# hbaatz/nerf-tex

Hardware: AMD Instinct MI355X
Metric: ray-samples/sec (MLP+composite) at 800x800x64 (higher is better)
Workload: dtype f32; 1 GPU; carpet 800x800x64: 640000 all-hit rays x 64 samples per GPU (BASELINE configs[1]), ParamNerf n_parameters=[1, 6], seeded glorot weights, inputs resident in HBM, fused PE+MLP+composite; rays_per_gpu=640000, hit_rays_total=640000, samples_per_ray=64

## Files before the change

### nerf_tex_amd/csrc/ntx_train.hip

```cpp
#include "nerftex.h"

#include <hip/hip_runtime.h>

#include <algorithm>
#include <cmath>
#include <cstdint>
#include <cstdio>
#include <cstdlib>
#include <cstring>
#include <type_traits>
#include <vector>

#include "ntx_train_device.h"

extern "C" int ntx_set_error(int code, const char *fmt, ...);

#define TRAIN_TRY(expr)                                                                                  \
    do {                                                                                                 \
        hipError_t e_ = (expr);                                                                          \
        if (e_ != hipSuccess) return ntx_set_error(NTX_E_HIP, "%s: %s", #expr, hipGetErrorString(e_)); \
    } while (0)

namespace ntx_train {

constexpr int TM = 128;

struct GemmArgs {
    const float *A; int lda; const float *B; int ldb; float *C; int ldc;
    int M, N, K;
    const float *bias;
    const float *mask; int ldmask;
    int relu, accumulate;
    int k_chunk; long long split_stride;
    float *colsum;
    int aligned;
};

template <int n, bool FAST>
__device__ __forceinline__ void fetch_run(const float *g, bool row_ok, int first, int bound, float *r, bool aligned_ok = false) {
    if (FAST) {
        const f32x4 *v = reinterpret_cast<const f32x4 *>(g);
#pragma unroll
        for (int q = 0; q < n / 4; ++q) { const f32x4 x = v[q]; r[4 * q] = x.x; r[4 * q + 1] = x.y; r[4 * q + 2] = x.z; r[4 * q + 3] = x.w; }
    } else if (row_ok && first + n <= bound && aligned_ok) {
        const f32x4 *v = reinterpret_cast<const f32x4 *>(g);
#pragma unroll
        for (int q = 0; q < n / 4; ++q) { const f32x4 x = v[q]; r[4 * q] = x.x; r[4 * q + 1] = x.y; r[4 * q + 2] = x.z; r[4 * q + 3] = x.w; }
    } else {
#pragma unroll
        for (int q = 0; q < n; ++q) r[q] = (row_ok && first + q < bound) ? g[q] : 0.0f;
    }
}

template <bool A_KCONTIG, int TN_, int TK_>
__device__ __forceinline__ void gemm_body(const GemmArgs &g, int bx, int by, int bz) {
    constexpr int THREADS = TN_ * 2, WCOLS = TN_ / 64, LROWA = TM + 4, LROWB_ = TN_ + 4;
    constexpr int FA = TM * TK_ / THREADS;
    constexpr int FB = TN_ * TK_ / THREADS;
    constexpr int TPR = THREADS / TK_;
    static_assert(FA % 4 == 0 && FB % 4 == 0 && FA * (THREADS / TM) == TK_ && TPR * FB == TN_ && TPR * FA == TM, "panel split");
    __shared__ __attribute__((aligned(16))) float As[2][TK_][LROWA], Bs[2][TK_][LROWB_];
    const int lane = threadIdx.x & 63, wave = threadIdx.x >> 6;
    const int j0 = bx * TN_, i0 = by * TM;
    const int k_begin = bz * g.k_chunk;
    const int k_end = k_begin + g.k_chunk < g.K ? k_begin + g.k_chunk : g.K;
    float *C = g.C + (size_t)bz * (size_t)g.split_stride;
    f32x16 acc[2][2];
#pragma unroll
    for (int a = 0; a < 2; ++a)
#pragma unroll
        for (int b = 0; b < 2; ++b)
#pragma unroll
            for (int r = 0; r < 16; ++r) acc[a][b][r] = 0.0f;
    float ra[2][FA], rb[2][FB], cs[FB];
#pragma unroll
    for (int q = 0; q < FB; ++q) cs[q] = 0.0f;
    const bool want_colsum = !A_KCONTIG && g.colsum != nullptr && by == 0;
    const bool inner = g.aligned && i0 + TM <= g.M && j0 + TN_ <= g.N;
    const int a_row = A_KCONTIG ? (int)(threadIdx.x % TM) : (int)(threadIdx.x / TPR), a_off = A_KCONTIG ? (int)(threadIdx.x / TM) * FA : (int)(threadIdx.x % TPR) * FA;
    const int b_row = (int)(threadIdx.x / TPR), b_off = (int)(threadIdx.x % TPR) * FB;
    auto fetch = [&](int k0, float *fa, float *fb) {
        const bool al = g.aligned != 0;
        if (A_KCONTIG) fetch_run<FA, false>(g.A + (size_t)(i0 + a_row) * g.lda + k0 + a_off, i0 + a_row < g.M, k0 + a_off, k_end, fa, al);
        else fetch_run<FA, false>(g.A + (size_t)(k0 + a_row) * g.lda + i0 + a_off, k0 + a_row < k_end, i0 + a_off, g.M, fa, al);
        fetch_run<FB, false>(g.B + (size_t)(k0 + b_row) * g.ldb + j0 + b_off, k0 + b_row < k_end, j0 + b_off, g.N, fb, al);
    };
    auto stash = [&](int buf, const float *fa, const float *fb) {
        if (want_colsum) {
#pragma unroll
            for (int q = 0; q < FB; ++q) cs[q] += fb[q];
        }
        if (A_KCONTIG) {
#pragma unroll
            for (int q = 0; q < FA; ++q) As[buf][a_off + q][a_row] = fa[q];
        } else {
            f32x4 *d = reinterpret_cast<f32x4 *>(&As[buf][a_row][a_off]);
#pragma unroll
            for (int q = 0; q < FA / 4; ++q) d[q] = f32x4{fa[4 * q], fa[4 * q + 1], fa[4 * q + 2], fa[4 * q + 3]};
        }
        f32x4 *d = reinterpret_cast<f32x4 *>(&Bs[buf][b_row][b_off]);
#pragma unroll
        for (int q = 0; q < FB / 4; ++q) d[q] = f32x4{fb[4 * q], fb[4 * q + 1], fb[4 * q + 2], fb[4 * q + 3]};
    };
    const int n_panels = (k_end - k_begin + TK_ - 1) / TK_;
    const int n_full = inner ? (k_end - k_begin) / TK_ : 0;
    const int wi = (wave / WCOLS) * 64 + 2 * (lane & 31), wj = (wave % WCOLS) * 64 + 2 * (lane & 31), kh = lane >> 5;
    const bool wave_live = j0 + (wave % WCOLS) * 64 < g.N;
    auto compute = [&](int buf) {
        if (!wave_live) return;
        f32x2 av[2], bv[2];
        av[0] = *reinterpret_cast<const f32x2 *>(&As[buf][kh][wi]); bv[0] = *reinterpret_cast<const f32x2 *>(&Bs[buf][kh][wj]);
#pragma unroll
        for (int st = 0; st < TK_ / 2; ++st) {
            const int c = st & 1, n = c ^ 1;
            if (st + 1 < TK_ / 2) {
                const int kk = 2 * (st + 1) + kh;
                av[n] = *reinterpret_cast<const f32x2 *>(&As[buf][kk][wi]); bv[n] = *reinterpret_cast<const f32x2 *>(&Bs[buf][kk][wj]);
            }
            __builtin_amdgcn_sched_barrier(0);
            acc[0][0] = __builtin_amdgcn_mfma_f32_32x32x2f32(av[c].x, bv[c].x, acc[0][0], 0, 0, 0);
            acc[0][1] = __builtin_amdgcn_mfma_f32_32x32x2f32(av[c].x, bv[c].y, acc[0][1], 0, 0, 0);
            acc[1][0] = __builtin_amdgcn_mfma_f32_32x32x2f32(av[c].y, bv[c].x, acc[1][0], 0, 0, 0);
            acc[1][1] = __builtin_amdgcn_mfma_f32_32x32x2f32(av[c].y, bv[c].y, acc[1][1], 0, 0, 0);
            __builtin_amdgcn_sched_barrier(0);
        }
    };
    auto fetch_fast = [&](int k0, float *fa, float *fb) {
        const float *ga = A_KCONTIG ? g.A + (size_t)(i0 + a_row) * g.lda + k0 + a_off : g.A + (size_t)(k0 + a_row) * g.lda + i0 + a_off;
        fetch_run<FA, true>(ga, true, 0, 0, fa);
        fetch_run<FB, true>(g.B + (size_t)(k0 + b_row) * g.ldb + j0 + b_off, true, 0, 0, fb);
    };
    auto pipeline = [&](auto fast_tag, int first, int last) {
        constexpr bool FAST = decltype(fast_tag)::value;
        auto get = [&](int kt, float *fa, float *fb) { if (FAST) fetch_fast(k_begin + kt * TK_, fa, fb); else fetch(k_begin + kt * TK_, fa, fb); };
        if (first >= last) return;
        get(first, ra[0], rb[0]); stash(0, ra[0], rb[0]);
        if (first + 1 < last) get(first + 1, ra[1], rb[1]);
        __syncthreads();
        int kt = first;
        for (; kt + 3 < last; kt += 2) {
            get(kt + 2, ra[0], rb[0]); compute(0); stash(1, ra[1], rb[1]); __syncthreads();
            get(kt + 3, ra[1], rb[1]); compute(1); stash(0, ra[0], rb[0]); __syncthreads();
        }
        for (; kt < last; ++kt) {
            const int buf = (kt - first) & 1;
            if (kt + 2 < last) { if (buf) get(kt + 2, ra[1], rb[1]); else get(kt + 2, ra[0], rb[0]); }
            compute(buf);
            if (kt + 1 < last) { if (buf) stash(0, ra[0], rb[0]); else stash(1, ra[1], rb[1]); }
            __syncthreads();
        }
    };
    pipeline(std::true_type{}, 0, n_full);
    pipeline(std::false_type{}, n_full, n_panels);
    const bool whole = i0 + TM <= g.M && j0 + TN_ <= g.N && (g.ldc % 2 == 0) && (!g.mask || g.ldmask % 2 == 0) && ((uintptr_t)C % 8 == 0) && ((uintptr_t)g.mask % 8 == 0);
    const int j = j0 + (wave % WCOLS) * 64 + 2 * (lane & 31);
    const float bj0 = (g.bias && j < g.N) ? g.bias[j] : 0.0f, bj1 = (g.bias && j + 1 < g.N) ? g.bias[j + 1] : 0.0f;
#pragma unroll
    for (int a = 0; a < 2; ++a)
#pragma unroll
        for (int r = 0; r < 16; ++r) {
            const int i = i0 + (wave / WCOLS) * 64 + 2 * (8 * (r >> 2) + (r & 3) + 4 * kh) + a;
            float v0 = acc[a][0][r], v1 = acc[a][1][r];
            float *c = C + (size_t)i * g.ldc + j;
            if (whole) {
                f32x2 *c2 = reinterpret_cast<f32x2 *>(c);
                if (g.accumulate) { const f32x2 o = *c2; v0 += o.x; v1 += o.y; }
                v0 += bj0; v1 += bj1;
                if (g.relu) { v0 = v0 > 0.0f ? v0 : 0.0f; v1 = v1 > 0.0f ? v1 : 0.0f; }
                if (g.mask) { const f32x2 mk = *reinterpret_cast<const f32x2 *>(g.mask + (size_t)i * g.ldmask + j); if (!(mk.x > 0.0f)) v0 = 0.0f; if (!(mk.y > 0.0f)) v1 = 0.0f; }
                *c2 = f32x2{v0, v1};
            } else if (i < g.M) {
#pragma unroll
                for (int b = 0; b < 2; ++b) {
                    if (j + b >= g.N) continue;
                    float v = b ? v1 : v0;
                    if (g.accumulate) v = v + c[b];
                    v = v + (b ? bj1 : bj0);
                    if (g.relu) v = v > 0.0f ? v : 0.0f;
                    if (g.mask && !(g.mask[(size_t)i * g.ldmask + j + b] > 0.0f)) v = 0.0f;
                    c[b] = v;
                }
            }
        }
    if (want_colsum) {
        float (*red)[LROWB_] = Bs[0];
#pragma unroll
        for (int q = 0; q < FB; ++q) red[b_row][b_off + q] = cs[q];
        __syncthreads();
        if ((int)threadIdx.x < TN_ && j0 + (int)threadIdx.x < g.N) {
            float sum = 0.0f;
            for (int q = 0; q < TK_; ++q) sum += red[q][threadIdx.x];
            g.colsum[(size_t)bz * g.N + j0 + threadIdx.x] = sum;
        }
    }
}


__device__ __forceinline__ void gemm_place(int lin, int nx, int ny, int nz, int &bx, int &by, int &bz) {
    const int tiles = nx * ny;
    if (nz % 8 == 0) {
        const int xcd = lin & 7, slot = lin >> 3, tile = slot % tiles;
        bz = (slot / tiles) * 8 + xcd; bx = tile % nx; by = tile / nx;
    } else { bx = lin % nx; by = (lin / nx) % ny; bz = lin / tiles; }
}
template <bool A_KCONTIG, int TN_, int TK_, int WAVES_PER_EU = 2>
__global__ __launch_bounds__(TN_ * 2) __attribute__((amdgpu_waves_per_eu(WAVES_PER_EU, 8))) void gemm_kernel(GemmArgs g) {
    int bx, by, bz;
    gemm_place(blockIdx.x + gridDim.x * (blockIdx.y + gridDim.y * blockIdx.z), gridDim.x, gridDim.y, gridDim.z, bx, by, bz);
    gemm_body<A_KCONTIG, TN_, TK_>(g, bx, by, bz);
}

constexpr int MAX_REDUCE_BATCH = 32;
struct ReduceJob { const float *partial; int n_split; long long stride, count, pair; float *out; long long first; };
struct ReduceBatch { ReduceJob job[MAX_REDUCE_BATCH]; int n; };
__global__ void reduce_batch_kernel(ReduceBatch b) {
    const long long g = (long long)blockIdx.x * blockDim.x + threadIdx.x;
    int j = 0;
    while (j + 1 < b.n && g >= b.job[j + 1].first) ++j;
    const ReduceJob &r = b.job[j];
    const long long e = g - r.first;
    if (e >= r.count) return;
    float s4[4] = {0.0f, 0.0f, 0.0f, 0.0f};
    auto at = [&](int z) { const float *p = r.partial + (size_t)z * r.stride + e; return r.pair > 0 ? p[0] + p[r.pair] : p[0]; };
    int z = 0;
    for (; z + 4 <= r.n_split; z += 4) {
#pragma unroll
        for (int q = 0; q < 4; ++q) s4[q] += at(z + q);
    }
    for (int q = 0; z < r.n_split; ++z, ++q) s4[q] += at(z);
    r.out[e] = (s4[0] + s4[1]) + (s4[2] + s4[3]);
}

enum { PACK_HIDDEN = 0, PACK_LINEAR = 1, PACK_AUX_ROW = 2, PACK_AUX_RGB = 3, PACK_COPY = 4 };
struct PackSeg {
    const float *src; long long sk, sc;
    int mode;
    int K, ncols, nt;
    float *dst; long long first, count;
};
struct PackArgs { const PackSeg *seg; int n_seg; long long total; };
__global__ void pack_kernel(PackArgs a) {
    const long long e = (long long)blockIdx.x * blockDim.x + threadIdx.x;
    if (e >= a.total) return;
    int lo = 0, hi = a.n_seg - 1;
    while (lo < hi) { const int mid = (lo + hi + 1) >> 1; if (a.seg[mid].first <= e) lo = mid; else hi = mid - 1; }
    const PackSeg &p = a.seg[lo];
    const long long o = e - p.first;
    float v = 0.0f;
    if (p.mode == PACK_COPY) v = p.src[o];
    else if (p.mode == PACK_AUX_ROW) {
        const int h = (int)(o >> 7) & 1, V = (int)(o & 127), k = hidden_row(V, h);
        v = k < p.K ? p.src[k * p.sk] : 0.0f;
    } else if (p.mode == PACK_AUX_RGB) {
        const int c = (int)(o >> 7), h = (int)(o >> 6) & 1, V = (int)(o & 63);
        v = p.src[hidden_row(V, h) * 3 + c];
    } else {
        const int c = (int)(o & 3), lane = (int)((o >> 2) & 63);
        const long long rec = o >> 8;
        const int G = p.nt / 4, g = (int)(rec % G), s = (int)(rec / G);
        const int f = lane & 31, kh = lane >> 5;
        const int k = p.mode == PACK_HIDDEN ? hidden_row(s, kh) : 2 * s + kh, col = 32 * (4 * g + c) + f;
        if (k < p.K && col < p.ncols) v = p.src[k * p.sk + col * p.sc];
    }
    p.dst[o] = v;
}

struct EncodeArgs {
    const float *rays_o, *rays_d, *z, *params, *cone;
    long long rays_per_param_row, M;
    int n_rays, S, n_geo, n_app, pos_freq, dir_freq, param_freq, blur_idx;
    float *posO; int ptiles;
    float *dirO; int dtiles;
    float *dists;
};
__global__ __launch_bounds__(64) void encode_kernel(EncodeArgs a) {
    const int lane = threadIdx.x, n = lane & 31, h = lane >> 5, blk = blockIdx.x, part = blockIdx.y;
    const long long m = (long long)blk * 32 + n;
    const bool valid = m < a.M;
    const int ray = valid ? (int)(m / a.S) : 0, s = valid ? (int)(m - (long long)ray * a.S) : 0;
    const float d[3] = {a.rays_d[3 * ray], a.rays_d[3 * ray + 1], a.rays_d[3 * ray + 2]};
    const float dn = sqrtf((d[0] * d[0] + d[1] * d[1]) + d[2] * d[2]);
    const float zr = a.z[(size_t)ray * a.S + s];
    const bool hit = isfinite(zr);
    const float z = hit ? zr : 0.0f;
    const int P = a.n_geo + a.n_app;
    const float *pr = a.params + (size_t)(ray / a.rays_per_param_row) * (P > 0 ? P : 1);
    auto param = [&](int c) { return c == a.blur_idx ? (hit ? pr[c] * (a.cone[ray] * z) : 0.0f) : pr[c]; };
    float *O = part == 0 ? a.posO : a.dirO;
    const int tiles = part == 0 ? a.ptiles : a.dtiles;
    auto put = [&](int row, float v) {
        if (!valid) v = 0.0f;
        O[(((size_t)blk * tiles + (row >> 5)) * 4 + (n >> 3)) * 256 + ((row & 31) + 32 * ((n >> 2) & 1)) * 4 + (n & 3)] = v;
    };
    auto fourier = [&](int r0, int D, int L, auto x) {
        if (h == 0) for (int c = 0; c < D; ++c) put(r0 + c, x(c));
        for (int f = 0; f < L; ++f)
            for (int c = 0; c < D; ++c) put(r0 + D + 2 * D * f + h * D + c, ntx::sin_q(ldexpf(1.0f, f) * x(c), h));
    };
    if (part == 0) {
        const float o[3] = {a.rays_o[3 * ray], a.rays_o[3 * ray + 1], a.rays_o[3 * ray + 2]};
        fourier(0, 3, a.pos_freq, [&](int c) { return o[c] + d[c] * z; });
        if (a.n_geo > 0) fourier(3 * (1 + 2 * a.pos_freq), a.n_geo, a.param_freq, [&](int c) { return param(c); });
    } else {
        fourier(0, 3, a.dir_freq, [&](int c) { return d[c] / dn; });
        if (a.n_app > 0) fourier(3 * (1 + 2 * a.dir_freq), a.n_app, a.param_freq, [&](int c) { return param(a.n_geo + c); });
        if (valid && h == 0) {
            const float zn = s + 1 < a.S ? a.z[(size_t)ray * a.S + s + 1] : 0.0f;
            const float dist = s + 1 < a.S ? zn - z : (a.S > 1 ? z - a.z[(size_t)ray * a.S + s - 1] : 0.0f);
            a.dists[(size_t)ray * a.S + s] = hit ? dist * dn : 0.0f;
        }
    }
}

__global__ __launch_bounds__(64) void encode_ipe_kernel(EncodeArgs a) {
    const int lane = threadIdx.x, n = lane & 31, h = lane >> 5, blk = blockIdx.x, part = blockIdx.y;
    const long long m = (long long)blk * 32 + n;
    const bool valid = m < a.M;
    const int ray = valid ? (int)(m / a.S) : 0, s = valid ? (int)(m - (long long)ray * a.S) : 0;
    const float d[3] = {a.rays_d[3 * ray], a.rays_d[3 * ray + 1], a.rays_d[3 * ray + 2]};
    const float dn = sqrtf((d[0] * d[0] + d[1] * d[1]) + d[2] * d[2]);
    const float *zr = a.z + (size_t)ray * (a.S + 1) + s;
    const float e0 = zr[0], e1 = zr[1];
    const bool hit = isfinite(e0) && isfinite(e1);
    const int P = a.n_geo + a.n_app;
    const float *pr = a.params + (size_t)(ray / a.rays_per_param_row) * (P + 1);
    auto param = [&](int k) { return pr[k < a.blur_idx ? k : k + 1]; };
    float *O = part == 0 ? a.posO : a.dirO;
    const int tiles = part == 0 ? a.ptiles : a.dtiles;
    auto put = [&](int row, float v) {
        if (!valid) v = 0.0f;
        O[(((size_t)blk * tiles + (row >> 5)) * 4 + (n >> 3)) * 256 + ((row & 31) + 32 * ((n >> 2) & 1)) * 4 + (n & 3)] = v;
    };
    auto fourier = [&](int r0, int D, int L, auto x) {
        if (h == 0) for (int c = 0; c < D; ++c) put(r0 + c, x(c));
        for (int f = 0; f < L; ++f)
            for (int c = 0; c < D; ++c) put(r0 + D + 2 * D * f + h * D + c, ntx::sin_q(ldexpf(1.0f, f) * x(c), h));
    };
    if (part == 0) {
        float mean[3] = {a.rays_o[3 * ray], a.rays_o[3 * ray + 1], a.rays_o[3 * ray + 2]}, cov[3] = {0.0f, 0.0f, 0.0f};
        if (hit) {
            float t_mean, t_var, r_var;
            ntx::cone_moments((e0 + e1) / 2.0f, (e1 - e0) / 2.0f, pr[a.blur_idx] * a.cone[ray], t_mean, t_var, r_var);
            for (int c = 0; c < 3; ++c) mean[c] = mean[c] + d[c] * t_mean;
            ntx::cone_cov(t_var, r_var, d, cov);
        }
        const int L = a.pos_freq;
        for (int f = 0; f < L; ++f)
            for (int c = 0; c < 3; ++c)
                put(h * 3 * L + 3 * f + c, ntx::sin_q(mean[c] * ldexpf(1.0f, f), h) * expf(-0.5f * (cov[c] * ldexpf(1.0f, 2 * f))));
        if (a.n_geo > 0) fourier(6 * L, a.n_geo, a.param_freq, [&](int c) { return param(c); });
    } else {
        fourier(0, 3, a.dir_freq, [&](int c) { return d[c] / dn; });
        if (a.n_app > 0) fourier(3 * (1 + 2 * a.dir_freq), a.n_app, a.param_freq, [&](int c) { return param(a.n_geo + c); });
        if (valid && h == 0) a.dists[(size_t)ray * a.S + s] = hit ? (e1 - e0) * dn : 0.0f;
    }
}

struct DirRowArgs {
    const float *rays_d, *params; long long rays_per_param_row;
    int n_rays, n_geo, n_app, dir_freq, param_freq, Kd, splice;
    const float *w, *bias;
    float *rows;
};
__global__ __launch_bounds__(256) void dirrow_kernel(DirRowArgs a) {
    __shared__ float feat[8 * MAX_PB_GROUPS];
    const int ray = blockIdx.x, f = threadIdx.x;
    const float d[3] = {a.rays_d[3 * ray], a.rays_d[3 * ray + 1], a.rays_d[3 * ray + 2]};
    const float dn = sqrtf((d[0] * d[0] + d[1] * d[1]) + d[2] * d[2]);
    const int P = a.n_geo + a.n_app + (a.splice >= 0 ? 1 : 0);
    const float *pr = a.params + (size_t)(ray / a.rays_per_param_row) * (P > 0 ? P : 1);
    if (f < a.Kd) {
        const int K3 = 3 * (1 + 2 * a.dir_freq);
        const int r = f < K3 ? f : f - K3, D = f < K3 ? 3 : a.n_app;
        auto x = [&](int c) { const int k = a.n_geo + c; return f < K3 ? d[c] / dn : pr[a.splice >= 0 && k >= a.splice ? k + 1 : k]; };
        float v;
        if (r < D) v = x(r);
        else { const int q = r - D, band = q / (2 * D), hc = q - band * 2 * D, hh = hc / D, c = hc - hh * D; v = ntx::sin_q(ldexpf(1.0f, band) * x(c), hh); }
        feat[f] = v;
    }
    __syncthreads();
    float acc = a.bias[f];
    for (int k = 0; k < a.Kd; ++k) acc = fmaf(feat[k], a.w[(size_t)k * 256 + f], acc);
    const int T = f >> 5, g = (f >> 3) & 3, h = (f >> 2) & 1, c = f & 3;
    a.rows[(size_t)ray * 256 + h * 128 + 16 * T + 4 * g + c] = acc;
}

struct CompositeArgs {
    const float *raw_rgb, *sigma, *dists;
    const float *noise;
    int n_rays, S, map_exr, composite_bkgd; float bkgd[3];
    const float *color_true, *alpha_true;
    int kind, loss_fn, alpha_loss_fn, filter_color_loss, use_hard_mask; float gamma;
    float *color, *alpha, *ray_loss;
    float *weights;
    float *dgrad;
    float *dhead;
    long long M;
};
constexpr int MAX_TRAIN_SAMPLES = 1024;
__device__ __forceinline__ float wave_sumf(float v) { for (int o = 32; o > 0; o >>= 1) v += __shfl_xor(v, o); return v; }
__device__ __forceinline__ float rgb_of(float raw, int map_exr) {
    if (map_exr) return raw > 0.0f ? raw + 1.0f : expf(raw);
    return 1.0f / (1.0f + expf(-raw));
}
__device__ __forceinline__ void loss_term(int fn, float t, float p, float inv_n, float &value, float &grad) {
    if (fn == NTX_LOSS_MSE) { const float e = t - p; value = e * e * inv_n; grad = -2.0f * e * inv_n; }
    else {
        const float e = t - p, den = (t + p) + 1e-2f, ae = fabsf(e);
        const float sgn = e > 0.0f ? 1.0f : (e < 0.0f ? -1.0f : 0.0f);
        value = ae / den * inv_n; grad = (-sgn / den - ae / (den * den)) * inv_n;
    }
}
__device__ __forceinline__ size_t dhead_at(long long m, int row) {
    const long long blk = m >> 5; const int p = (int)(m & 31);
    return (size_t)((blk * 4 + (p >> 3)) * 256 + (row + 32 * ((p >> 2) & 1)) * 4 + (p & 3));
}
__global__ __launch_bounds__(256) void composite_loss_kernel(CompositeArgs a) {
    __shared__ float sh_a[4][MAX_TRAIN_SAMPLES], sh_T[4][MAX_TRAIN_SAMPLES];
    const int lane = threadIdx.x & 63, wave = threadIdx.x >> 6;
    if (blockIdx.x == 0) {
        const long long end = (a.M + 31) / 32 * 32;
        for (long long m = a.M + threadIdx.x; m < end; m += 256)
            for (int r = 0; r < 4; ++r) a.dhead[dhead_at(m, r)] = 0.0f;
    }
    const int ray = blockIdx.x * 4 + wave;
    if (ray >= a.n_rays) return;
    const int S = a.S;
    const float *sg = a.sigma + (size_t)ray * S, *ds = a.dists + (size_t)ray * S, *rr = a.raw_rgb + (size_t)ray * S * 3;
    const float *nz = a.noise ? a.noise + (size_t)ray * S : nullptr;
    float *el = sh_a[wave], *T = sh_T[wave];
    for (int s = lane; s < S; s += 64) { const float v = nz ? sg[s] + nz[s] : sg[s]; const float r = v > 0.0f ? v : 0.0f; el[s] = expf(-r * ds[s]); }
    __builtin_amdgcn_wave_barrier();
    float carry = 1.0f;
    for (int s0 = 0; s0 < S; s0 += 64) {
        const int s = s0 + lane;
        float f = s < S ? el[s] + 1e-10f : 1.0f, incl = f;
        for (int o = 1; o < 64; o <<= 1) { const float w = __shfl_up(incl, o); if (lane >= o) incl *= w; }
        float excl = __shfl_up(incl, 1);
        if (lane == 0) excl = 1.0f;
        if (s < S) T[s] = carry * excl;
        carry *= __shfl(incl, 63);
    }
    __builtin_amdgcn_wave_barrier();
    float c0 = 0.0f, c1 = 0.0f, c2 = 0.0f, A = 0.0f;
    for (int s = lane; s < S; s += 64) {
        const float w = (1.0f - el[s]) * T[s];
        c0 += w * rgb_of(rr[3 * s], a.map_exr); c1 += w * rgb_of(rr[3 * s + 1], a.map_exr); c2 += w * rgb_of(rr[3 * s + 2], a.map_exr);
        A += w;
        if (a.weights) a.weights[(size_t)ray * S + s] = w;
    }
    c0 = wave_sumf(c0); c1 = wave_sumf(c1); c2 = wave_sumf(c2); A = wave_sumf(A);
    if (a.composite_bkgd) { c0 += (1.0f - A) * a.bkgd[0]; c1 += (1.0f - A) * a.bkgd[1]; c2 += (1.0f - A) * a.bkgd[2]; }
    const float cp[3] = {c0, c1, c2};
    float dC[3], dA = 0.0f, total = 0.0f;
    {
        const float inv_c = 1.0f / (float)(a.n_rays * 3), inv_a = 1.0f / (float)a.n_rays;
        float mask = 1.0f;
        if (a.kind == NTX_LOSS_ALPHA && a.filter_color_loss) mask = a.use_hard_mask ? (a.alpha_true[ray] > 0.0f ? 1.0f : 0.0f) : a.alpha_true[ray];
        for (int c = 0; c < 3; ++c) {
            float v, gr;
            loss_term(a.loss_fn, a.color_true[3 * ray + c] * mask, cp[c] * mask, inv_c, v, gr);
            total += v; dC[c] = gr * mask;
        }
        if (a.kind == NTX_LOSS_ALPHA) { float v; loss_term(a.alpha_loss_fn, a.alpha_true[ray], A, inv_a, v, dA); total += a.gamma * v; dA *= a.gamma; }
    }
    if (lane == 0) { a.color[3 * ray] = c0; a.color[3 * ray + 1] = c1; a.color[3 * ray + 2] = c2; a.alpha[ray] = A; a.ray_loss[ray] = total; }
    if (a.composite_bkgd) dA -= (dC[0] * a.bkgd[0] + dC[1] * a.bkgd[1]) + dC[2] * a.bkgd[2];
    float Z_carry = 1.0f, V_carry = 0.0f;
    for (int s0 = ((S - 1) / 64) * 64; s0 >= 0; s0 -= 64) {
        const int s = s0 + lane;
        float cs = 0.0f, rgb[3] = {0.0f, 0.0f, 0.0f}, e = 1.0f;
        float F = 1.0f, Bz = 0.0f, Bv = 0.0f;
        if (s < S) {
            e = el[s];
            for (int c = 0; c < 3; ++c) rgb[c] = rgb_of(rr[3 * s + c], a.map_exr);
            cs = (dC[0] * rgb[0] + dC[1] * rgb[1]) + dC[2] * rgb[2];
            F = e + 1e-10f; Bz = -1e-10f; Bv = cs * (1.0f - e);
        }
        for (int o = 1; o < 64; o <<= 1) {
            const float Fo = __shfl_down(F, o), Bzo = __shfl_down(Bz, o), Bvo = __shfl_down(Bv, o);
            if (lane + o < 64) { Bz = fmaf(F, Bzo, Bz); Bv = fmaf(F, Bvo, Bv); F *= Fo; }
        }
        float Fn = __shfl_down(F, 1), Bzn = __shfl_down(Bz, 1), Bvn = __shfl_down(Bv, 1);
        if (lane == 63) { Fn = 1.0f; Bzn = 0.0f; Bvn = 0.0f; }
        const float Z = fmaf(Fn, Z_carry, Bzn), V = fmaf(Fn, V_carry, Bvn);
        if (s < S) {
            const float w = (1.0f - e) * T[s];
            const float d_a = T[s] * fmaf(dA, Z, cs - V);
            const float sig = nz ? sg[s] + nz[s] : sg[s];
            float gr[4];
            for (int c = 0; c < 3; ++c) {
                const float raw = rr[3 * s + c];
                const float drgb = a.map_exr ? (raw > 0.0f ? 1.0f : expf(raw)) : rgb[c] * (1.0f - rgb[c]);
                gr[c] = w * dC[c] * drgb;
            }
            gr[3] = sig > 0.0f ? d_a * ds[s] * e : 0.0f;
            const long long m = (long long)ray * S + s;
            *reinterpret_cast<f32x4 *>(a.dgrad + 4 * m) = f32x4{gr[0], gr[1], gr[2], gr[3]};
            for (int r = 0; r < 4; ++r) a.dhead[dhead_at(m, r)] = gr[r];
        }
        const float F0 = __shfl(F, 0);
        Z_carry = fmaf(F0, Z_carry, __shfl(Bz, 0)); V_carry = fmaf(F0, V_carry, __shfl(Bv, 0));
    }
}
__global__ __launch_bounds__(1024) void loss_sum_kernel(const float *__restrict__ ray_loss, int n_rays, float *__restrict__ loss) {
    __shared__ float red[1024];
    float total = 0.0f;
    for (int r = threadIdx.x; r < n_rays; r += blockDim.x) total += ray_loss[r];
    red[threadIdx.x] = total;
    __syncthreads();
    for (int o = blockDim.x / 2; o > 0; o >>= 1) { if ((int)threadIdx.x < o) red[threadIdx.x] += red[threadIdx.x + o]; __syncthreads(); }
    if (threadIdx.x == 0) *loss = red[0];
}

__global__ void adam_kernel(float *__restrict__ w, const float *__restrict__ g, float *__restrict__ m, float *__restrict__ v, long long n, float lr_t, float b1,
                            float b2, float eps) {
    const long long e = (long long)blockIdx.x * blockDim.x + threadIdx.x;
    if (e >= n) return;
    const float ge = g[e];
    const float me = m[e] + (ge - m[e]) * (1.0f - b1);
    const float ve = v[e] + (ge * ge - v[e]) * (1.0f - b2);
    m[e] = me; v[e] = ve;
    w[e] = w[e] - (me * lr_t) / (sqrtf(ve) + eps);
}

}

struct TLayer { int in, out; size_t w, b; };

struct ntx_trainer {
    int device = 0, cus = 256;
    ntx_model_desc desc{};
    int Kp = 0, Kd = 0, P = 0, ptiles = 0, dtiles = 0, PS = 0, DS = 0;
    bool ipe = false;
    TLayer trunk[8], feature, c1, c2, rgb, alpha;
    size_t n_weights = 0;
    long long cap = 0, cap_blocks = 0, cap_rays = 0;
    float *w = nullptr, *grad = nullptr, *adam_m = nullptr, *adam_v = nullptr;
    float *wfwd = nullptr, *wdx = nullptr, *aux = nullptr; size_t fwd_floats = 0, dx_floats = 0;
    ntx_train::PackSeg *pack_seg = nullptr; int n_pack = 0; long long pack_total = 0;
    float *posO = nullptr, *dirO = nullptr;
    float *act = nullptr; long long act_stride = 0;
    unsigned int *bits = nullptr; long long bits_stride = 0;
    int fwd_variant = 0;
    float *sigma = nullptr, *raw_rgb = nullptr, *z = nullptr, *dists = nullptr, *noise = nullptr;
    float *dirrow = nullptr;
    float *dgrad = nullptr, *dhead = nullptr, *gout = nullptr; long long gout_stride = 0;
    ntx_train::DwJob *jobs = nullptr; int n_jobs = 0; long long total_cost = 0;
    std::vector<ntx_train::DwJob> jobs_host; std::vector<int> reduce_job;
    float *dw_partial = nullptr;
    ntx_train::ReduceBatch reduce{};
    float *color = nullptr, *alpha_out = nullptr, *ray_loss = nullptr, *loss = nullptr;
    float *weights_out = nullptr;
    float *stash = nullptr;
    long long adam_iterations = 0;
};

namespace {

using namespace ntx_train;


void free_all(ntx_trainer *t) {
    if (!t) return;
    (void)hipSetDevice(t->device);
    void *ptrs[] = {t->w, t->grad, t->adam_m, t->adam_v, t->wfwd, t->wdx, t->aux, t->pack_seg, t->posO, t->dirO, t->sigma, t->raw_rgb, t->z, t->dists, t->noise,
                    t->dgrad, t->dhead, t->jobs, t->dw_partial, t->stash, t->dirrow, t->color, t->alpha_out, t->ray_loss, t->loss, t->act, t->bits, t->gout};
    for (void *p : ptrs) if (p) (void)hipFree(p);
    delete t;
}

template <bool AK>
void launch_gemm(hipStream_t st, GemmArgs g) {
    g.k_chunk = g.K;
    g.aligned = (g.lda % 4 == 0) && (g.ldb % 4 == 0) && (((uintptr_t)g.A | (uintptr_t)g.B) % 16 == 0);
    hipLaunchKernelGGL((gemm_kernel<AK, 128, 16>), dim3((g.N + 127) / 128, (g.M + TM - 1) / TM, 1), dim3(256), 0, st, g);
}

}

namespace ntx_train {
template <int K, bool HOIST> void launch_fwd_variant(hipStream_t st, unsigned grid, const FwdArgs &a);
void launch_fwd_chain(int variant, bool hoist, hipStream_t st, unsigned grid, const FwdArgs &a) {
    switch (variant * 2 + (hoist ? 1 : 0)) {
        case 0: launch_fwd_variant<0, false>(st, grid, a); break;
        case 1: launch_fwd_variant<0, true>(st, grid, a); break;
        case 2: launch_fwd_variant<1, false>(st, grid, a); break;
        case 3: launch_fwd_variant<1, true>(st, grid, a); break;
        case 4: launch_fwd_variant<2, false>(st, grid, a); break;
        case 5: launch_fwd_variant<2, true>(st, grid, a); break;
        case 6: launch_fwd_variant<3, false>(st, grid, a); break;
        default: launch_fwd_variant<3, true>(st, grid, a); break;
    }
}
}

extern "C" {

int ntx_sample_depths(const float *t, int64_t n_rays, int n_points, uint32_t flags, uint64_t perturb_seed, const ntx_render_opts *opts, float *z_out,
                      ntx_stream stream);
int ntx_sample_noise(int64_t n_rays, int n_points, uint64_t seed, const ntx_render_opts *opts, float *noise_out, ntx_stream stream);

int ntx_trainer_create(const ntx_model_desc *desc, const float *weights, size_t n_floats, int device, int64_t max_rays, int max_samples_per_ray, ntx_trainer **out) {
    if (!out) return ntx_set_error(NTX_E_INVALID, "out is NULL");
    *out = nullptr;
    if (!desc || !weights) return ntx_set_error(NTX_E_INVALID, "desc / weights is NULL");
    const bool ipe = desc->pos_encoding == NTX_POS_IPE && desc->n_pos == 6;
    if (desc->kind != NTX_MODEL_PARAMNERF || desc->depth != 8 || desc->width != 256 || desc->skip != 4 || desc->color_depth != 1 ||
        !((desc->pos_encoding == NTX_POS_FOURIER && desc->n_pos == 3) || ipe))
        return ntx_set_error(NTX_E_UNSUPPORTED, "training is built for the ParamNerf architecture of the shipped training configs (depth 8, width 256, skips [4], color_depth 1, "
                                                "Fourier features on n_pos 3 or IPE on n_pos 6); others render but do not train");
    if (desc->n_geo < 0 || desc->n_app < 0 || desc->n_geo + desc->n_app > 16) return ntx_set_error(NTX_E_INVALID, "n_parameters out of range");
    if (desc->pos_freq < 0 || desc->dir_freq < 0 || desc->param_freq < 0) return ntx_set_error(NTX_E_INVALID, "negative band count");
    const int Kp = (ipe ? 6 * desc->pos_freq : 3 * (1 + 2 * desc->pos_freq)) + desc->n_geo * (1 + 2 * desc->param_freq), Kd = 3 * (1 + 2 * desc->dir_freq) + desc->n_app * (1 + 2 * desc->param_freq);
    if (Kp > 8 * MAX_PB_GROUPS || Kd > 8 * MAX_PB_GROUPS)
        return ntx_set_error(NTX_E_UNSUPPORTED, "training: pos_map (%d) / dir_map (%d) wider than %d features (the chain holds a block's encoded inputs in registers)", Kp, Kd,
                             8 * MAX_PB_GROUPS);
    if (max_rays < 1 || max_samples_per_ray < 2 || max_samples_per_ray > MAX_TRAIN_SAMPLES || max_rays * (int64_t)max_samples_per_ray > (int64_t)1 << 30)
        return ntx_set_error(NTX_E_INVALID, "max_rays / max_samples_per_ray out of range (samples per ray <= %d)", MAX_TRAIN_SAMPLES);
    int ndev = 0;
    if (hipGetDeviceCount(&ndev) != hipSuccess || ndev <= 0) return ntx_set_error(NTX_E_NODEVICE, "no HIP device visible");
    if (device < 0 || device >= ndev) return ntx_set_error(NTX_E_INVALID, "device %d out of range [0,%d)", device, ndev);
    ntx_trainer *t = new ntx_trainer();
    t->device = device; t->desc = *desc; t->ipe = ipe;
    t->P = desc->n_geo + desc->n_app; t->Kp = Kp; t->Kd = Kd;
    t->ptiles = (Kp + 31) / 32; t->dtiles = (Kd + 31) / 32;
    {
        const int psg = ((Kp + 1) / 2 + 3) / 4, dsg = ((Kd + 1) / 2 + 3) / 4;
        t->fwd_variant = 3;
        for (int v = 2; v >= 0; --v)
            if (FWD_VARIANTS[v][0] >= psg && FWD_VARIANTS[v][1] >= dsg &&
                FWD_VARIANTS[v][0] + FWD_VARIANTS[v][1] <= FWD_VARIANTS[t->fwd_variant][0] + FWD_VARIANTS[t->fwd_variant][1]) t->fwd_variant = v;
        t->PS = 4 * FWD_VARIANTS[t->fwd_variant][0]; t->DS = 4 * FWD_VARIANTS[t->fwd_variant][1];
    }
    size_t p = 0;
    auto take = [&](int in, int o) { TLayer l{in, o, p, p + (size_t)in * o}; p += (size_t)in * o + o; return l; };
    int k = Kp;
    for (int i = 0; i < 8; ++i) { t->trunk[i] = take(k, 256); k = 256 + (i == 4 ? Kp : 0); }
    t->feature = take(256, 256); t->c1 = take(256 + Kd, 256); t->c2 = take(256, 128); t->rgb = take(128, 3); t->alpha = take(256, 1);
    t->n_weights = p;
    if (n_floats != p) { delete t; return ntx_set_error(NTX_E_INVALID, "weights: %zu floats, the model has %zu", n_floats, p); }
    const long long M = (long long)max_rays * max_samples_per_ray, NB = (M + 31) / 32;
    t->cap = M; t->cap_rays = max_rays; t->cap_blocks = NB;
    int rc = hipSetDevice(device) == hipSuccess ? NTX_OK : ntx_set_error(NTX_E_HIP, "hipSetDevice(%d) failed", device);
    if (rc == NTX_OK) { int n = 0; if (hipDeviceGetAttribute(&n, hipDeviceAttributeMultiprocessorCount, device) == hipSuccess && n > 0) t->cus = n; }
    auto alloc = [&](float **d, size_t n, bool zero = false) -> int {
        if (rc != NTX_OK) return rc;
        if (hipMalloc((void **)d, (n ? n : 1) * sizeof(float)) != hipSuccess) return rc = ntx_set_error(NTX_E_HIP, "hipMalloc of %zu floats failed", n);
        if (zero && hipMemset(*d, 0, (n ? n : 1) * sizeof(float)) != hipSuccess) return rc = ntx_set_error(NTX_E_HIP, "hipMemset failed");
        return rc;
    };
    alloc(&t->w, p); alloc(&t->grad, p, true); alloc(&t->adam_m, p, true); alloc(&t->adam_v, p, true);
    alloc(&t->posO, (size_t)NB * t->ptiles * 1024, true); alloc(&t->dirO, (size_t)NB * t->dtiles * 1024, true);
    t->act_stride = t->gout_stride = NB * 8 * 1024; t->bits_stride = NB * 256;
    alloc(&t->act, (size_t)t->act_stride * 11); alloc((float **)&t->bits, (size_t)t->bits_stride * 10); alloc(&t->gout, (size_t)t->gout_stride * 11);
    auto act = [&](int i) { return t->act + (size_t)i * t->act_stride; };
    auto gout = [&](int i) { return t->gout + (size_t)i * t->gout_stride; };
    alloc(&t->sigma, (size_t)M); alloc(&t->raw_rgb, (size_t)M * 3); alloc(&t->z, (size_t)(M + max_rays)); alloc(&t->dists, (size_t)M); alloc(&t->noise, (size_t)M);
    alloc(&t->dirrow, (size_t)max_rays * 256);
    alloc(&t->dgrad, (size_t)NB * 32 * 4); alloc(&t->dhead, (size_t)NB * 1024, true);
    alloc(&t->color, (size_t)max_rays * 3); alloc(&t->alpha_out, (size_t)max_rays); alloc(&t->ray_loss, (size_t)max_rays); alloc(&t->loss, 1);
    if (rc == NTX_OK && hipMemcpy(t->w, weights, p * sizeof(float), hipMemcpyHostToDevice) != hipSuccess) rc = ntx_set_error(NTX_E_HIP, "weight upload failed");
    std::vector<PackSeg> segs;
    long long first = 0;
    auto seg = [&](const float *src, long long sk, long long sc, int mode, int K, int ncols, int nt, size_t *stream_floats, int nsteps) {
        PackSeg s{}; s.src = src; s.sk = sk; s.sc = sc; s.mode = mode; s.K = K; s.ncols = ncols; s.nt = nt;
        const int ring = stream_floats == &t->dx_floats ? DX_RING : RING;
        const long long recs = ((long long)nsteps * (nt / 4) + ring - 1) / ring * ring;
        s.count = recs * 256; s.first = first; s.dst = (float *)(uintptr_t)(*stream_floats * sizeof(float));
        first += s.count; *stream_floats += (size_t)s.count;
        segs.push_back(s);
    };
    const float *W = t->w;
    auto fwd_hidden = [&](const TLayer &l, int row0, int nt) { seg(W + l.w + (size_t)row0 * l.out, l.out, 1, PACK_HIDDEN, 256, l.out, nt, &t->fwd_floats, 128); };
    auto fwd_linear = [&](const TLayer &l, int K, int nsteps) { seg(W + l.w, l.out, 1, PACK_LINEAR, K, l.out, 8, &t->fwd_floats, nsteps); };
    fwd_linear(t->trunk[0], Kp, t->PS);
    for (int i = 1; i < 8; ++i) {
        if (i == 5) { fwd_linear(t->trunk[5], Kp, t->PS); fwd_hidden(t->trunk[5], Kp, 8); }
        else fwd_hidden(t->trunk[i], 0, 8);
    }
    fwd_hidden(t->feature, 0, 8);
    fwd_linear(t->c1, Kd, t->DS); fwd_hidden(t->c1, Kd, 8);
    fwd_hidden(t->c2, 0, 4);
    const size_t n_fwd_segs = segs.size();
    auto dx_hidden = [&](const TLayer &l, int row0, int K, int nsteps) { seg(W + l.w + (size_t)row0 * l.out, 1, l.out, PACK_HIDDEN, K, 256, 8, &t->dx_floats, nsteps); };
    seg(W + t->rgb.w, 1, 3, PACK_LINEAR, 3, 128, 4, &t->dx_floats, 2);
    dx_hidden(t->c2, 0, 128, 64);
    dx_hidden(t->c1, Kd, 256, 128);
    dx_hidden(t->feature, 0, 256, 128);
    seg(W + t->alpha.w, 1, 1, PACK_LINEAR, 1, 256, 8, &t->dx_floats, 1);
    for (int i = 7; i >= 1; --i) dx_hidden(t->trunk[i], i == 5 ? Kp : 0, 256, 128);
    const size_t n_stream_segs = segs.size();
    auto tail = [&](size_t of, size_t *stream_floats) { PackSeg s = segs[of]; s.count = (long long)(stream_floats == &t->dx_floats ? DX_RING : RING) * 256; s.first = first; s.dst = (float *)(uintptr_t)(*stream_floats * sizeof(float));
                                                        first += s.count; *stream_floats += (size_t)s.count; segs.push_back(s); };
    tail(0, &t->fwd_floats); tail(n_fwd_segs, &t->dx_floats);
    auto aux_seg = [&](const float *src, int mode, int K, long long count, size_t at) {
        PackSeg s{}; s.src = src; s.sk = 1; s.mode = mode; s.K = K; s.count = count; s.first = first; s.dst = (float *)(uintptr_t)(at * sizeof(float));
        first += count; segs.push_back(s);
    };
    for (int i = 0; i < 8; ++i) aux_seg(W + t->trunk[i].b, PACK_AUX_ROW, 256, 256, AUX_BIAS + (size_t)i * 256);
    aux_seg(W + t->feature.b, PACK_AUX_ROW, 256, 256, AUX_BIAS + 8 * 256); aux_seg(W + t->c1.b, PACK_AUX_ROW, 256, 256, AUX_BIAS + 9 * 256);
    aux_seg(W + t->c2.b, PACK_AUX_ROW, 128, 256, AUX_BIAS + 10 * 256);
    aux_seg(W + t->alpha.w, PACK_AUX_ROW, 256, 256, AUX_ALPHA_W); aux_seg(W + t->alpha.b, PACK_COPY, 1, 1, AUX_ALPHA_B);
    aux_seg(W + t->rgb.w, PACK_AUX_RGB, 128, 384, AUX_RGB_W); aux_seg(W + t->rgb.b, PACK_COPY, 3, 3, AUX_RGB_B);
    t->pack_total = first; t->n_pack = (int)segs.size();
    alloc(&t->wfwd, t->fwd_floats); alloc(&t->wdx, t->dx_floats); alloc(&t->aux, AUX_FLOATS, true);
    if (rc == NTX_OK) {
        for (size_t i = 0; i < segs.size(); ++i) {
            const bool is_aux = i >= n_stream_segs + 2, is_fwd = i < n_fwd_segs || i == n_stream_segs;
            float *base = is_aux ? t->aux : is_fwd ? t->wfwd : t->wdx;
            segs[i].dst = (float *)((char *)base + (uintptr_t)segs[i].dst);
        }
        if (hipMalloc((void **)&t->pack_seg, segs.size() * sizeof(PackSeg)) != hipSuccess ||
            hipMemcpy(t->pack_seg, segs.data(), segs.size() * sizeof(PackSeg), hipMemcpyHostToDevice) != hipSuccess)
            rc = ntx_set_error(NTX_E_HIP, "segment table upload failed");
    }
    std::vector<DwJob> &jobs = t->jobs_host;
    struct RJ { int job; long long at, count, pair; size_t out; };
    std::vector<RJ> rjobs;
    auto new_job = [&]() { DwJob j{}; for (DwWave &w : j.w) w.shape = -1; jobs.push_back(j); return (int)jobs.size() - 1; };
    auto matrix = [&](int j, int K, int N, size_t g_kernel, long long g_bias, long long *at_bias) {
        const long long at = jobs[j].slot_floats;
        jobs[j].slot_floats += (long long)K * N;
        rjobs.push_back(RJ{j, at, (long long)K * N, 0, g_kernel});
        *at_bias = -1;
        if (g_bias >= 0) { *at_bias = jobs[j].slot_floats; jobs[j].slot_floats += 2 * N; rjobs.push_back(RJ{j, *at_bias, N, N, (size_t)g_bias}); }
        return at;
    };
    auto wave = [&](int j, int w, int shape, const float *A, int rtA, int a0, const float *B, int rtB, int b0, long long at, int K, int N, int c_lo, long long at_bias) {
        DwWave &d = jobs[j].w[w];
        d.A = A; d.rtA = rtA; d.a0 = a0; d.B = B; d.rtB = rtB; d.b0 = b0; d.shape = shape; d.out = at; d.ldc = N; d.row0 = a0 * 32; d.rows_valid = K;
        d.col0 = b0 * 32; d.c_lo = c_lo; d.c_hi = c_lo + N; d.bias_out = a0 == 0 ? at_bias : -1;
        const int cost = shape == 0 ? 256 : shape == 1 ? 198 : 68;
        if (cost > jobs[j].cost) jobs[j].cost = cost;
    };
    auto layer_job = [&](const float *X, const float *dY, size_t g_kernel, size_t g_bias) {
        const int j = new_job(); long long ab; const long long at = matrix(j, 256, 256, g_kernel, (long long)g_bias, &ab);
        for (int w = 0; w < 4; ++w) wave(j, w, 0, X, 8, 4 * (w >> 1), dY, 8, 4 * (w & 1), at, 256, 256, 0, ab);
    };
    {
        const TLayer &r = t->rgb, &al = t->alpha, &c2 = t->c2, &c1 = t->c1, &f = t->feature;
        for (int i = 7; i >= 1; --i) layer_job(act(i - 1), gout(10 - i), t->trunk[i].w + (size_t)(i == 5 ? Kp : 0) * 256, t->trunk[i].b);
        layer_job(act(7), gout(2), f.w, f.b);
        layer_job(act(8), gout(1), c1.w + (size_t)Kd * 256, c1.b);
        {
            const int j = new_job(); long long ab0, ab5;
            const long long at0 = matrix(j, Kp, 256, t->trunk[0].w, (long long)t->trunk[0].b, &ab0), at5 = matrix(j, Kp, 256, t->trunk[5].w, -1, &ab5);
            for (int w = 0; w < 2; ++w) { wave(j, w, 1, t->posO, t->ptiles, 0, gout(10), 8, 4 * w, at0, Kp, 256, 0, ab0); wave(j, 2 + w, 1, t->posO, t->ptiles, 0, gout(5), 8, 4 * w, at5, Kp, 256, 0, ab5); }
        }
        {
            const int j = new_job(); long long abd, ab2;
            const long long atd = matrix(j, Kd, 256, c1.w, -1, &abd), at2 = matrix(j, 256, 128, c2.w, (long long)c2.b, &ab2);
            for (int w = 0; w < 2; ++w) { wave(j, w, 1, t->dirO, t->dtiles, 0, gout(1), 8, 4 * w, atd, Kd, 256, 0, abd); wave(j, 2 + w, 0, act(9), 8, 4 * w, gout(0), 4, 0, at2, 256, 128, 0, ab2); }
        }
        {
            const int j = new_job(); long long abr, aba;
            const long long atr = matrix(j, 128, 3, r.w, (long long)r.b, &abr), ata = matrix(j, 256, 1, al.w, (long long)al.b, &aba);
            wave(j, 0, 2, act(10), 4, 0, t->dhead, 1, 0, atr, 128, 3, 0, abr);
            for (int w = 0; w < 2; ++w) wave(j, 1 + w, 2, act(7), 8, 4 * w, t->dhead, 1, 0, ata, 256, 1, 3, aba);
        }
    }
    t->n_jobs = (int)jobs.size();
    size_t partial_floats = 0;
    for (DwJob &j : jobs) {
        t->total_cost += j.cost;
    }
    for (DwJob &j : jobs) {
        const long long slots = ((long long)j.cost * t->cus + t->total_cost - 1) / t->total_cost + 2;
        j.first_float = (long long)partial_floats; partial_floats += (size_t)(slots * j.slot_floats);
    }
    alloc(&t->dw_partial, partial_floats);
    if (rc == NTX_OK) {
        if (hipMalloc((void **)&t->jobs, jobs.size() * sizeof(DwJob)) != hipSuccess ||
            hipMemcpy(t->jobs, jobs.data(), jobs.size() * sizeof(DwJob), hipMemcpyHostToDevice) != hipSuccess)
            rc = ntx_set_error(NTX_E_HIP, "job table upload failed");
        if ((int)rjobs.size() > MAX_REDUCE_BATCH) rc = ntx_set_error(NTX_E_INVALID, "trainer: too many weight gradients for one launch");
        long long rfirst = 0;
        for (size_t i = 0; i < rjobs.size() && rc == NTX_OK; ++i) {
            ReduceJob &r = t->reduce.job[t->reduce.n++];
            const DwJob &j = jobs[rjobs[i].job];
            r.partial = t->dw_partial + j.first_float + rjobs[i].at; r.n_split = 0; r.stride = j.slot_floats; r.count = rjobs[i].count; r.pair = rjobs[i].pair;
            r.out = t->grad + rjobs[i].out; r.first = rfirst;
            rfirst += (rjobs[i].count + 255) / 256 * 256;
            t->reduce_job.push_back(rjobs[i].job);
        }
    }
    if (rc != NTX_OK) { free_all(t); return rc; }
    *out = t;
    return NTX_OK;
}

int ntx_trainer_destroy(ntx_trainer *t) { free_all(t); return NTX_OK; }

size_t ntx_trainer_weight_count(const ntx_trainer *t) { return t ? t->n_weights : 0; }

static float *trainer_vector(ntx_trainer *t, int what) {
    return what == NTX_TRAINER_WEIGHTS ? t->w : what == NTX_TRAINER_GRADIENTS ? t->grad : what == NTX_TRAINER_ADAM_M ? t->adam_m : what == NTX_TRAINER_ADAM_V ? t->adam_v : nullptr;
}

int ntx_trainer_get(ntx_trainer *t, int what, float *out_host, size_t n_floats) {
    if (!t || !out_host) return ntx_set_error(NTX_E_INVALID, "NULL argument");
    if (n_floats != t->n_weights) return ntx_set_error(NTX_E_INVALID, "%zu floats asked, the model has %zu", n_floats, t->n_weights);
    const float *src = trainer_vector(t, what);
    if (!src) return ntx_set_error(NTX_E_INVALID, "what = %d", what);
    TRAIN_TRY(hipSetDevice(t->device));
    TRAIN_TRY(hipDeviceSynchronize());
    TRAIN_TRY(hipMemcpy(out_host, src, n_floats * sizeof(float), hipMemcpyDeviceToHost));
    return NTX_OK;
}

int ntx_trainer_activation(ntx_trainer *t, int layer, int64_t n_samples_total, float *out_host) {
    if (!t || !out_host) return ntx_set_error(NTX_E_INVALID, "NULL argument");
    if (n_samples_total < 1 || n_samples_total > t->cap) return ntx_set_error(NTX_E_INVALID, "n_samples_total out of range");
    const float *src = nullptr; int tiles = 8;
    auto act = [&](int i) { return t->act + (size_t)i * t->act_stride; };
    auto gout = [&](int i) { return t->gout + (size_t)i * t->gout_stride; };
    if (layer >= 0 && layer < 8) src = act(layer);
    else if (layer == 8) src = act(9);
    else if (layer == 9) { src = act(10); tiles = 4; }
    else if (layer == 10) src = t->sigma;
    else if (layer >= 20 && layer < 28) src = gout(10 - (layer - 20));
    else if (layer == 28) src = gout(1);
    else if (layer == 29) src = gout(2);
    else if (layer == 11) src = t->raw_rgb;
    else if (layer == 30) src = t->dgrad;
    else return ntx_set_error(NTX_E_INVALID, "layer %d (0-7 trunk, 8 / 9 the colour layers, 10 the density, 11 the raw colour; 20-29 the kept gradients, 30 the composite's adjoint)", layer);
    TRAIN_TRY(hipSetDevice(t->device));
    TRAIN_TRY(hipDeviceSynchronize());
    if (layer == 10 || layer == 11 || layer == 30) {
        const size_t width = layer == 10 ? 1 : (layer == 11 ? 3 : 4);
        TRAIN_TRY(hipMemcpy(out_host, src, (size_t)n_samples_total * width * sizeof(float), hipMemcpyDeviceToHost)); return NTX_OK;
    }
    const long long nb = (n_samples_total + 31) / 32;
    std::vector<float> tmp((size_t)nb * tiles * 1024);
    TRAIN_TRY(hipMemcpy(tmp.data(), src, tmp.size() * sizeof(float), hipMemcpyDeviceToHost));
    const int width = tiles * 32;
    for (long long m = 0; m < n_samples_total; ++m) {
        const long long blk = m >> 5; const int p = (int)(m & 31);
        const float *rec = tmp.data() + ((size_t)blk * tiles * 4 + (p >> 3)) * 256 + 32 * ((p >> 2) & 1) * 4 + (p & 3);
        float *o = out_host + (size_t)m * width;
        for (int T = 0; T < tiles; ++T)
            for (int i = 0; i < 32; ++i) o[32 * T + i] = rec[(size_t)T * 1024 + i * 4];
    }
    return NTX_OK;
}

int ntx_trainer_set_weights(ntx_trainer *t, const float *weights_host, size_t n_floats) { return ntx_trainer_set(t, NTX_TRAINER_WEIGHTS, weights_host, n_floats); }

int ntx_trainer_set(ntx_trainer *t, int what, const float *values_host, size_t n_floats) {
    if (!t || !values_host) return ntx_set_error(NTX_E_INVALID, "NULL argument");
    if (n_floats != t->n_weights) return ntx_set_error(NTX_E_INVALID, "%zu floats given, the model has %zu", n_floats, t->n_weights);
    float *dst = trainer_vector(t, what);
    if (!dst) return ntx_set_error(NTX_E_INVALID, "what = %d", what);
    TRAIN_TRY(hipSetDevice(t->device));
    TRAIN_TRY(hipDeviceSynchronize());
    TRAIN_TRY(hipMemcpy(dst, values_host, n_floats * sizeof(float), hipMemcpyHostToDevice));
    return NTX_OK;
}

int ntx_trainer_set_iterations(ntx_trainer *t, int64_t iterations) {
    if (!t || iterations < 0) return ntx_set_error(NTX_E_INVALID, "trainer is NULL or iterations < 0");
    t->adam_iterations = iterations;
    return NTX_OK;
}

int ntx_trainer_composite_weights(ntx_trainer *t, float *weights_dev) {
    if (!t) return ntx_set_error(NTX_E_INVALID, "trainer is NULL");
    if (t->ipe && weights_dev) return ntx_set_error(NTX_E_UNSUPPORTED, "an IPE trainer has no importance pass (MipRenderer: renderer.py:403-404)");
    t->weights_out = weights_dev;
    return NTX_OK;
}

namespace ntx_train {
__global__ void add_kernel(float *__restrict__ dst, const float *__restrict__ src, long long n) {
    const long long e = (long long)blockIdx.x * blockDim.x + threadIdx.x;
    if (e < n) dst[e] += src[e];
}
}

int ntx_trainer_stash_gradients(ntx_trainer *t, int op, ntx_stream stream) {
    if (!t || (op != 0 && op != 1)) return ntx_set_error(NTX_E_INVALID, "trainer is NULL or op is not 0 (keep) / 1 (add back)");
    TRAIN_TRY(hipSetDevice(t->device));
    if (!t->stash) {
        if (op == 1) return ntx_set_error(NTX_E_INVALID, "no gradient was kept");
        TRAIN_TRY(hipMalloc((void **)&t->stash, t->n_weights * sizeof(float)));
    }
    if (op == 0) TRAIN_TRY(hipMemcpyAsync(t->stash, t->grad, t->n_weights * sizeof(float), hipMemcpyDeviceToDevice, (hipStream_t)stream));
    else hipLaunchKernelGGL(ntx_train::add_kernel, dim3((unsigned)((t->n_weights + 255) / 256)), dim3(256), 0, (hipStream_t)stream, t->grad, t->stash, (long long)t->n_weights);
    TRAIN_TRY(hipGetLastError());
    return NTX_OK;
}

int ntx_trainer_device_weights(ntx_trainer *t, const float **weights_dev) {
    if (!t || !weights_dev) return ntx_set_error(NTX_E_INVALID, "NULL argument");
    *weights_dev = t->w;
    return NTX_OK;
}

int ntx_trainer_allreduce_gradients(ntx_trainer *t, ntx_comm *comm, ntx_stream stream) {
    if (!t || !comm) return ntx_set_error(NTX_E_INVALID, "NULL argument");
    return ntx_allreduce_mean_f32(comm, t->grad, t->n_weights, stream);
}

int ntx_train_step_gradients(ntx_trainer *t, const float *rays_o, const float *rays_d, const float *tnear_far, const float *params, int64_t rays_per_param_row,
                             const float *cone_scale, int64_t n_rays, int n_samples, int blur_idx, uint32_t flags, const float *bkgd, uint64_t perturb_seed,
                             const ntx_render_opts *opts, const float *z_vals, const float *color_true, const float *alpha_true, const ntx_loss_desc *loss,
                             float *color_pred, float *alpha_pred, float *loss_out, ntx_stream stream) {
    if (!t) return ntx_set_error(NTX_E_INVALID, "trainer is NULL");
    const int P_in = t->P + (t->ipe ? 1 : 0);
    if (!rays_o || !rays_d || (!tnear_far && !z_vals) || !color_true || !loss || (P_in > 0 && !params)) return ntx_set_error(NTX_E_INVALID, "NULL buffer");
    if (n_rays < 1 || n_rays > t->cap_rays || n_samples < 2 || (long long)n_rays * n_samples > t->cap) return ntx_set_error(NTX_E_INVALID, "n_rays x n_samples beyond what the trainer was created for");
    if (n_samples > MAX_TRAIN_SAMPLES) return ntx_set_error(NTX_E_INVALID, "n_samples > %d", MAX_TRAIN_SAMPLES);
    if (blur_idx >= P_in || (blur_idx >= 0 && !cone_scale) || (t->ipe && blur_idx < 0)) return ntx_set_error(NTX_E_INVALID, "bad blur_idx / cone_scale");
    if (loss->size < sizeof(ntx_loss_desc) || (loss->kind != NTX_LOSS_NERF && loss->kind != NTX_LOSS_ALPHA) || (loss->loss_fn != NTX_LOSS_MSE && loss->loss_fn != NTX_LOSS_SMAPE) ||
        (loss->alpha_loss_fn != NTX_LOSS_MSE && loss->alpha_loss_fn != NTX_LOSS_SMAPE))
        return ntx_set_error(NTX_E_INVALID, "bad ntx_loss_desc");
    if (loss->kind == NTX_LOSS_ALPHA && !alpha_true) return ntx_set_error(NTX_E_INVALID, "AlphaLoss needs alpha_true");
    if (rays_per_param_row < 1) rays_per_param_row = 1;
    TRAIN_TRY(hipSetDevice(t->device));
    hipStream_t st = (hipStream_t)stream;
    const long long M = (long long)n_rays * n_samples;
    const int S = n_samples, n_blocks = (int)((M + 31) / 32);
    {
        PackArgs pa{t->pack_seg, t->n_pack, t->pack_total};
        hipLaunchKernelGGL(pack_kernel, dim3((unsigned)((t->pack_total + 255) / 256)), dim3(256), 0, st, pa);
    }
    const float *z = z_vals;
    if (!z) {
        int rc = ntx_sample_depths(tnear_far, n_rays, t->ipe ? S + 1 : S, flags & NTX_FLAG_PERTURB, perturb_seed, opts, t->z, stream);
        if (rc != NTX_OK) return rc;
        z = t->z;
    }
    const float *noise = nullptr;
    if (flags & NTX_FLAG_RAW_NOISE) {
        int rc = ntx_sample_noise(n_rays, S, perturb_seed, opts, t->noise, stream);
        if (rc != NTX_OK) return rc;
        noise = t->noise;
    }
    {
        EncodeArgs e{}; e.rays_o = rays_o; e.rays_d = rays_d; e.z = z; e.params = params; e.cone = cone_scale; e.rays_per_param_row = rays_per_param_row; e.M = M;
        e.n_rays = (int)n_rays; e.S = S; e.n_geo = t->desc.n_geo; e.n_app = t->desc.n_app; e.pos_freq = t->desc.pos_freq; e.dir_freq = t->desc.dir_freq;
        e.param_freq = t->desc.param_freq; e.blur_idx = blur_idx; e.posO = t->posO; e.ptiles = t->ptiles; e.dirO = t->dirO;
        e.dtiles = t->dtiles; e.dists = t->dists;
        if (t->ipe) hipLaunchKernelGGL(encode_ipe_kernel, dim3((unsigned)n_blocks, 2), dim3(64), 0, st, e);
        else hipLaunchKernelGGL(encode_kernel, dim3((unsigned)n_blocks, 2), dim3(64), 0, st, e);
    }
    const unsigned chain_grid = (unsigned)std::min<long long>(t->cus, (n_blocks + 3) / 4);
    {
        FwdArgs f{}; f.stream = t->wfwd; f.stream_bytes = (uint32_t)(t->fwd_floats * sizeof(float)); f.aux = t->aux; f.M = M;
        f.ptiles = t->ptiles; f.dtiles = t->dtiles; f.pos = t->posO; f.dir = t->dirO;
        f.act = t->act; f.act_stride = t->act_stride; f.bits = t->bits; f.bits_stride = t->bits_stride;
        f.sigma = t->sigma; f.raw_rgb = t->raw_rgb;
        const bool hoist = (t->ipe || blur_idx < 0 || blur_idx < t->desc.n_geo) && S % 32 == 0 && getenv("NERFTEX_TRAIN_NO_DIR_HOIST") == nullptr;
        if (hoist) {
            DirRowArgs dr{}; dr.rays_d = rays_d; dr.params = params; dr.rays_per_param_row = rays_per_param_row; dr.n_rays = (int)n_rays; dr.n_geo = t->desc.n_geo;
            dr.n_app = t->desc.n_app; dr.dir_freq = t->desc.dir_freq; dr.param_freq = t->desc.param_freq; dr.Kd = t->Kd; dr.w = t->w + t->c1.w; dr.bias = t->w + t->c1.b;
            dr.rows = t->dirrow; dr.splice = t->ipe ? blur_idx : -1;
            hipLaunchKernelGGL(dirrow_kernel, dim3((unsigned)n_rays), dim3(256), 0, st, dr);
        }
        f.dirrow = t->dirrow; f.n_rays = (int)n_rays; f.S = S;
        launch_fwd_chain(t->fwd_variant, hoist, st, chain_grid, f);
    }
    {
        CompositeArgs c{};
        c.raw_rgb = t->raw_rgb; c.sigma = t->sigma; c.dists = t->dists; c.noise = noise; c.n_rays = (int)n_rays; c.S = S; c.map_exr = (flags & NTX_FLAG_MAP_EXR) ? 1 : 0;
        c.composite_bkgd = (flags & NTX_FLAG_COMPOSITE_BKGD) ? 1 : 0;
        for (int k = 0; k < 3; ++k) c.bkgd[k] = bkgd ? bkgd[k] : 1.0f;
        c.color_true = color_true; c.alpha_true = alpha_true; c.kind = loss->kind; c.loss_fn = loss->loss_fn; c.alpha_loss_fn = loss->alpha_loss_fn;
        c.filter_color_loss = loss->filter_color_loss; c.use_hard_mask = loss->use_hard_mask; c.gamma = loss->gamma;
        c.weights = t->weights_out;
        c.color = color_pred ? color_pred : t->color; c.alpha = alpha_pred ? alpha_pred : t->alpha_out; c.ray_loss = t->ray_loss; c.dgrad = t->dgrad; c.dhead = t->dhead; c.M = M;
        hipLaunchKernelGGL(composite_loss_kernel, dim3((unsigned)((n_rays + 3) / 4)), dim3(256), 0, st, c);
        hipLaunchKernelGGL(loss_sum_kernel, dim3(1), dim3(1024), 0, st, t->ray_loss, (int)n_rays, loss_out ? loss_out : t->loss);
    }
    {
        DxArgs d{}; d.stream = t->wdx; d.stream_bytes = (uint32_t)(t->dx_floats * sizeof(float)); d.M = M; d.dgrad = t->dgrad;
        d.out = t->gout; d.out_stride = t->gout_stride; d.bits = t->bits; d.bits_stride = t->bits_stride;
        launch_dx_chain(st, chain_grid, d);
    }
    {
        DwArgs d{}; d.jobs = t->jobs; d.n_jobs = t->n_jobs; d.n_blocks = n_blocks; d.total_cost = t->total_cost; d.partial = t->dw_partial;
        const long long G = t->cus, W = t->total_cost * n_blocks;
#ifdef NTX_TRAIN_CLOCKS
        static unsigned long long *clocks = nullptr;
        const size_t nck = (size_t)G * (2 + 3 * t->n_jobs);
        if (getenv("NERFTEX_DW_CLOCKS")) {
            if (!clocks) (void)hipMalloc((void **)&clocks, nck * sizeof(unsigned long long));
            (void)hipMemsetAsync(clocks, 0, nck * sizeof(unsigned long long), st);
            d.clocks = clocks;
        }
#endif
        launch_dw(st, (unsigned)G, d);
#ifdef NTX_TRAIN_CLOCKS
        if (d.clocks) {
            std::vector<unsigned long long> h(nck);
            (void)hipStreamSynchronize(st);
            (void)hipMemcpy(h.data(), clocks, nck * sizeof(unsigned long long), hipMemcpyDeviceToHost);
            unsigned long long t0 = ~0ull;
            for (long long g = 0; g < G; ++g) t0 = std::min(t0, h[g * (2 + 3 * t->n_jobs)]);
            FILE *f = fopen(getenv("NERFTEX_DW_CLOCKS"), "w");
            if (f) {
                for (long long g = 0; g < G; ++g) {
                    const unsigned long long *c = &h[g * (2 + 3 * t->n_jobs)];
                    fprintf(f, "%lld %llu %llu", g, c[0] - t0, c[1] - t0);
                    for (int j = 0; j < t->n_jobs; ++j) if (c[4 + 3 * j]) fprintf(f, "  j%d cost %d blocks %llu %llu-%llu", j, t->jobs_host[j].cost, c[2 + 3 * j], c[3 + 3 * j] - t0, c[4 + 3 * j] - t0);
                    fprintf(f, "\n");
                }
                fclose(f);
            }
        }
#endif
        ReduceBatch rb = t->reduce;
        std::vector<int> slots(t->n_jobs);
        long long start = 0;
        for (int j = 0; j < t->n_jobs; ++j) {
            const long long span = (long long)t->jobs_host[j].cost * n_blocks;
            slots[j] = (int)(dw_last_g(G, W, start, span) - dw_first_g(G, W, start) + 1);
            start += span;
        }
        for (int i = 0; i < rb.n; ++i) rb.job[i].n_split = slots[t->reduce_job[i]];
        const long long total = rb.job[rb.n - 1].first + (rb.job[rb.n - 1].count + 255) / 256 * 256;
        hipLaunchKernelGGL(reduce_batch_kernel, dim3((unsigned)(total / 256)), dim3(256), 0, st, rb);
    }
    TRAIN_TRY(hipGetLastError());
    return NTX_OK;
}

int ntx_trainer_adam_step(ntx_trainer *t, float lrate, float lrate_decay_steps, float lrate_decay_rate, float beta_1, float beta_2, float epsilon, ntx_stream stream) {
    if (!t) return ntx_set_error(NTX_E_INVALID, "trainer is NULL");
    TRAIN_TRY(hipSetDevice(t->device));
    const double step = (double)t->adam_iterations;
    double lr = lrate;
    if (lrate_decay_steps > 0) lr = (double)lrate * std::pow((double)lrate_decay_rate, step / (double)lrate_decay_steps);
    const double tt = step + 1.0;
    const float lr_t = (float)((double)(float)lr * std::sqrt(1.0 - std::pow((double)beta_2, tt)) / (1.0 - std::pow((double)beta_1, tt)));
    hipLaunchKernelGGL(ntx_train::adam_kernel, dim3((unsigned)((t->n_weights + 255) / 256)), dim3(256), 0, (hipStream_t)stream, t->w, t->grad, t->adam_m, t->adam_v,
                       (long long)t->n_weights, lr_t, beta_1, beta_2, epsilon);
    t->adam_iterations += 1;
    TRAIN_TRY(hipGetLastError());
    return NTX_OK;
}

int64_t ntx_trainer_iterations(const ntx_trainer *t) { return t ? t->adam_iterations : -1; }

int ntx_gemm_f32(const float *A, int lda, int a_kcontig, const float *B, int ldb, int b_kcontig, float *C, int ldc, int M, int N, int K, const float *bias, int relu,
                 ntx_stream stream) {
    if (!A || !B || !C || M < 1 || N < 1 || K < 1) return ntx_set_error(NTX_E_INVALID, "bad GEMM arguments");
    ntx_train::GemmArgs g{}; g.A = A; g.lda = lda; g.B = B; g.ldb = ldb; g.C = C; g.ldc = ldc; g.M = M; g.N = N; g.K = K; g.bias = bias; g.relu = relu;
    hipStream_t st = (hipStream_t)stream;
    if (b_kcontig) return ntx_set_error(NTX_E_UNSUPPORTED, "B must be [K][N]");
    if (a_kcontig) launch_gemm<true>(st, g); else launch_gemm<false>(st, g);
    TRAIN_TRY(hipGetLastError());
    return NTX_OK;
}

}
```

### nerf_tex_amd/csrc/ntx_train_device.h

```cpp
#pragma once

#include "ntx_device.h"

namespace ntx_train {

using ntx::f32x16;
using ntx::f32x4;
using ntx::hidden_row;
using ntx::mfma32;
using ntx::RING;
using ntx::static_for;
typedef float f32x2 __attribute__((ext_vector_type(2)));
typedef int i32x4 __attribute__((ext_vector_type(4)));
typedef unsigned int u32x4 __attribute__((ext_vector_type(4)));

#define TRN_DEV __device__ __forceinline__

TRN_DEV __amdgpu_buffer_rsrc_t make_rsrc(const void *base, long long bytes) {
    const long long b = bytes < 0 ? 0 : (bytes > 0x7ffffff0ll ? 0x7ffffff0ll : bytes);
    return __builtin_amdgcn_make_buffer_rsrc(const_cast<void *>(base), 0, (int)b, 0x00020000);
}

TRN_DEV uint32_t o_lane_bytes(int lane) {
    const int n = lane & 31, h = lane >> 5;
    return (uint32_t)((n >> 3) * 1024 + ((n >> 2) & 1) * 512 + h * 64 + (n & 3) * 4);
}
constexpr int STORE_NT = 0;
constexpr uint32_t o_value_bytes(int V) { return (uint32_t)((V >> 4) * 4096 + ((V & 15) >> 2) * 128 + (V & 3) * 16); }

template <int R>
struct WRingT {
    static constexpr int DEPTH = R;
    __amdgpu_buffer_rsrc_t rsrc;
    uint32_t voff;
    f32x4 r[R];
};
typedef WRingT<RING> WRing;
constexpr int DX_RING = 16;
template <class WR>
TRN_DEV f32x4 wr_load(const WR &w, uint32_t byte_off) {
#ifdef NTX_X_WSMALL
    byte_off &= 0xffffu;
#endif
#ifdef NTX_X_NOWLOAD
    if (byte_off >= (uint32_t)WR::DEPTH * 1024u) return w.r[(byte_off >> 10) % WR::DEPTH];
#endif
    return __builtin_bit_cast(f32x4, __builtin_amdgcn_raw_buffer_load_b128(w.rsrc, w.voff, byte_off, 0));
}

template <int NSTEPS, int NMT, bool ZERO, class WR, class Extra>
TRN_DEV void seg_hidden(f32x16 (&acc)[8], WR &ws, uint32_t &sbase, const float (&hin)[128], Extra &&extra) {
    constexpr int RPS = NMT / 4, RING = WR::DEPTH;
    static_assert((NSTEPS * RPS) % RING == 0, "whole ring turns");
    const f32x16 zero = {0.f, 0.f, 0.f, 0.f, 0.f, 0.f, 0.f, 0.f, 0.f, 0.f, 0.f, 0.f, 0.f, 0.f, 0.f, 0.f};
    static_for<NSTEPS>([&](auto S) {
        constexpr int s = S;
        f32x4 w;
        static_for<NMT>([&](auto MT) {
            constexpr int mt = MT;
            if constexpr (mt % 4 == 0) {
                constexpr int rec = s * RPS + mt / 4;
                w = ws.r[rec % RING];
                ws.r[rec % RING] = wr_load(ws, sbase + (uint32_t)(rec + RING) * 1024u);
            }
            if constexpr (ZERO && s == 0) acc[mt] = mfma32(w[mt % 4], hin[s], zero);
            else acc[mt] = mfma32(w[mt % 4], hin[s], acc[mt]);
            extra(S, MT);
            __builtin_amdgcn_sched_barrier(0);
        });
    });
    sbase += (uint32_t)(NSTEPS * RPS) * 1024u;
}

template <int NG, class Fetch>
TRN_DEV void seg_mem(f32x16 (&acc)[8], WRing &ws, uint32_t &sbase, float (&pb)[12], Fetch &&fetch) {
    static_assert(RING == 8, "a group of 4 k-steps of 8 tiles is one ring turn");
    static_for<NG>([&](auto G) {
        constexpr int g = G;
        if constexpr (g + 2 < NG) fetch(std::integral_constant<int, g + 2>{});
        static_for<4>([&](auto K) {
            constexpr int k = K;
            f32x4 w;
            static_for<8>([&](auto MT) {
                constexpr int mt = MT;
                if constexpr (mt % 4 == 0) {
                    constexpr int slot = 2 * k + mt / 4;
                    w = ws.r[slot];
                    ws.r[slot] = wr_load(ws, sbase + (uint32_t)(8 * g + slot + RING) * 1024u);
                }
                acc[mt] = mfma32(w[mt % 4], pb[4 * (g % 3) + k], acc[mt]);
                __builtin_amdgcn_sched_barrier(0);
            });
        });
    });
    sbase += (uint32_t)NG * 8192u;
}

template <int NKS, int NMT, bool ZERO, class WR>
TRN_DEV void seg_few(f32x16 (&acc)[8], WR &ws, uint32_t &sbase, const float (&b)[NKS]) {
    constexpr int RPS = NMT / 4, RING = WR::DEPTH;
    static_assert(NKS * RPS <= RING, "one ring turn");
    const f32x16 zero = {0.f, 0.f, 0.f, 0.f, 0.f, 0.f, 0.f, 0.f, 0.f, 0.f, 0.f, 0.f, 0.f, 0.f, 0.f, 0.f};
    static_for<RING>([&](auto I) {
        constexpr int rec = I;
        const f32x4 w = ws.r[rec];
        ws.r[rec] = wr_load(ws, sbase + (uint32_t)(rec + RING) * 1024u);
        if constexpr (rec < NKS * RPS) {
            constexpr int s = rec / RPS, t0 = 4 * (rec % RPS);
            static_for<4>([&](auto C) {
                constexpr int c = C;
                if constexpr (ZERO && s == 0) acc[t0 + c] = mfma32(w[c], b[s], zero);
                else acc[t0 + c] = mfma32(w[c], b[s], acc[t0 + c]);
                __builtin_amdgcn_sched_barrier(0);
            });
        }
    });
    sbase += (uint32_t)RING * 1024u;
}

template <int V0>
TRN_DEV void convert8_relu_bits(float (&hin)[128], const f32x16 (&prev)[8], uint32_t &w) {
    constexpr int T = V0 >> 4, R = V0 & 15;
    float t0, t1, t2, t3;
    asm("v_accvgpr_read_b32 %0, %13\n\tv_accvgpr_read_b32 %1, %14\n\tv_accvgpr_read_b32 %2, %15\n\tv_accvgpr_read_b32 %3, %16\n\t"
        "v_accvgpr_read_b32 %4, %17\n\tv_accvgpr_read_b32 %5, %18\n\tv_accvgpr_read_b32 %6, %19\n\tv_accvgpr_read_b32 %7, %20\n\t"
        "v_sub_f32 %9, 0, %0\n\tv_sub_f32 %10, 0, %1\n\tv_sub_f32 %11, 0, %2\n\tv_sub_f32 %12, 0, %3\n\t"
        "v_alignbit_b32 %8, %8, %9, 31\n\tv_alignbit_b32 %8, %8, %10, 31\n\tv_alignbit_b32 %8, %8, %11, 31\n\tv_alignbit_b32 %8, %8, %12, 31\n\t"
        "v_sub_f32 %9, 0, %4\n\tv_sub_f32 %10, 0, %5\n\tv_sub_f32 %11, 0, %6\n\tv_sub_f32 %12, 0, %7\n\t"
        "v_alignbit_b32 %8, %8, %9, 31\n\tv_alignbit_b32 %8, %8, %10, 31\n\tv_alignbit_b32 %8, %8, %11, 31\n\tv_alignbit_b32 %8, %8, %12, 31\n\t"
        "v_max_f32 %0, 0, %0\n\tv_max_f32 %1, 0, %1\n\tv_max_f32 %2, 0, %2\n\tv_max_f32 %3, 0, %3\n\t"
        "v_max_f32 %4, 0, %4\n\tv_max_f32 %5, 0, %5\n\tv_max_f32 %6, 0, %6\n\tv_max_f32 %7, 0, %7"
        : "=&v"(hin[V0 + 0]), "=&v"(hin[V0 + 1]), "=&v"(hin[V0 + 2]), "=&v"(hin[V0 + 3]), "=&v"(hin[V0 + 4]), "=&v"(hin[V0 + 5]), "=&v"(hin[V0 + 6]),
          "=&v"(hin[V0 + 7]), "+v"(w), "=&v"(t0), "=&v"(t1), "=&v"(t2), "=&v"(t3)
        : "a"(prev[T][R + 0]), "a"(prev[T][R + 1]), "a"(prev[T][R + 2]), "a"(prev[T][R + 3]), "a"(prev[T][R + 4]), "a"(prev[T][R + 5]), "a"(prev[T][R + 6]),
          "a"(prev[T][R + 7]));
}
constexpr int keep_bit(int V) { return 31 - (V & 31); }

template <int NMT>
TRN_DEV void convert_relu_bits(float (&hin)[128], const f32x16 (&prev)[8], u32x4 &bits) {
    static_for<(NMT + 1) / 2>([&](auto W) {
        constexpr int wd = W;
        uint32_t w = 0;
        static_for<(NMT - 2 * wd >= 2 ? 4 : 2)>([&](auto Q) { convert8_relu_bits<32 * wd + 8 * decltype(Q)::value>(hin, prev, w); });
        bits[wd] = w;
    });
}
template <int NMT>
TRN_DEV void convert_linear(float (&hin)[128], const f32x16 (&prev)[8]) {
    static_for<NMT * 16>([&](auto V) { constexpr int v = V; hin[v] = prev[v >> 4][v & 15]; });
}
template <int NMT>
TRN_DEV void convert_mask(float (&hin)[128], const f32x16 (&prev)[8], const u32x4 &bits) {
    static_for<NMT * 16>([&](auto V) {
        constexpr int v = V;
        const float x = prev[v >> 4][v & 15];
        const int keep = __builtin_amdgcn_sbfe((int)bits[v >> 5], keep_bit(v), 1);
        hin[v] = __builtin_bit_cast(float, __builtin_bit_cast(int, x) & keep);
    });
}

constexpr int AUX_BIAS = 0, AUX_ALPHA_W = 11 * 256, AUX_ALPHA_B = AUX_ALPHA_W + 256, AUX_RGB_W = AUX_ALPHA_B + 4, AUX_RGB_B = AUX_RGB_W + 384,
              AUX_FLOATS = AUX_RGB_B + 4;
template <int MT>
TRN_DEV void bias_tile(f32x16 (&acc)[8], const float *aux, int layer, int h) {
    const f32x4 *b = reinterpret_cast<const f32x4 *>(aux + AUX_BIAS + layer * 256 + h * 128) + MT * 4;
    const f32x4 v0 = b[0], v1 = b[1], v2 = b[2], v3 = b[3];
    acc[MT] = f32x16{v0.x, v0.y, v0.z, v0.w, v1.x, v1.y, v1.z, v1.w, v2.x, v2.y, v2.z, v2.w, v3.x, v3.y, v3.z, v3.w};
}

constexpr int MAX_PB_GROUPS = 12;
struct FwdArgs {
    const float *stream; uint32_t stream_bytes;
    const float *aux;
    long long M;
    int ptiles, dtiles;
    const float *pos, *dir;
    float *act; long long act_stride;
    unsigned int *bits; long long bits_stride;
    float *sigma, *raw_rgb;
    const float *dirrow; int n_rays, S;
};

#ifdef NTX_TRAIN_FWD
template <int PSG, int DSG, bool HOIST>
__global__ __launch_bounds__(256) __attribute__((amdgpu_waves_per_eu(1, 1))) void fwd_chain_kernel(FwdArgs a) {
    __shared__ __attribute__((aligned(16))) float aux_lds[AUX_FLOATS];
    __shared__ __attribute__((aligned(16))) float rows_lds[HOIST ? 4 * 256 : 4];
    ntx::load_aux(aux_lds, a.aux, AUX_FLOATS);
    const int lane = threadIdx.x & 63, n = lane & 31, h = lane >> 5;
    const int wave = __builtin_amdgcn_readfirstlane(blockIdx.x * 4 + (threadIdx.x >> 6)), nwaves = gridDim.x * 4;
    const int n_blocks = (int)((a.M + 31) >> 5);
    if (wave >= n_blocks) return;
    WRing ws;
    ws.rsrc = make_rsrc(a.stream, a.stream_bytes);
    ws.voff = (uint32_t)lane * 16u;
    static_for<RING>([&](auto I) { ws.r[I] = wr_load(ws, (uint32_t)decltype(I)::value * 1024u); });
    const uint32_t lane_o = o_lane_bytes(lane), lane_r = (uint32_t)((n >> 3) * 1024 + ((n >> 2) & 1) * 512 + (n & 3) * 4 + h * 16), lane16 = (uint32_t)lane * 16u;
    float pb[12];
    const __amdgpu_buffer_rsrc_t rs_row = make_rsrc(a.dirrow, HOIST ? (long long)a.n_rays * 1024 : 0);
    __amdgpu_buffer_rsrc_t rs_in = make_rsrc(a.pos + (size_t)wave * a.ptiles * 1024, (long long)a.ptiles * 4096);
    auto fetch = [&](auto G) {
        constexpr int g = G;
        static_for<4>([&](auto K) {
            constexpr int k = K;
            constexpr int s = 4 * g + k;
            pb[4 * (g % 3) + k] = __builtin_bit_cast(float, __builtin_amdgcn_raw_buffer_load_b32(rs_in, lane_r, (uint32_t)((s >> 4) * 4096 + (s & 15) * 32), 0));
        });
    };
    fetch(std::integral_constant<int, 0>{}); fetch(std::integral_constant<int, 1>{});
    for (int blk = wave; blk < n_blocks; blk += nwaves) {
        uint32_t opaque_zero = 0;
        asm volatile("" : "+v"(opaque_zero));
        const float *aux = aux_lds + opaque_zero;
        const float *rows_aux = rows_lds + opaque_zero + (HOIST ? (threadIdx.x >> 6) * 256 : 0) - AUX_BIAS - 9 * 256;
        uint32_t sbase = 0;
        f32x16 acc[8];
        float hin[128];
        const long long m = (long long)blk * 32 + n;
        const bool valid = m < a.M;
        if constexpr (HOIST) {
            const uint32_t ray = __builtin_amdgcn_readfirstlane((int)(((uint32_t)blk * 32u) / (uint32_t)a.S));
            const f32x4 x0 = __builtin_bit_cast(f32x4, __builtin_amdgcn_raw_buffer_load_b128(rs_row, lane16, (ray < (uint32_t)a.n_rays ? ray : (uint32_t)a.n_rays - 1u) * 1024u, 0));
            *reinterpret_cast<f32x4 *>(rows_lds + (threadIdx.x >> 6) * 256 + lane * 4) = x0;
            __builtin_amdgcn_wave_barrier();
        }
        __amdgpu_buffer_rsrc_t rs_out = make_rsrc(a.act, 0);
        auto leaves_to = [&](int idx, int tiles) { rs_out = make_rsrc(a.act + (size_t)idx * a.act_stride + (size_t)blk * tiles * 1024, (long long)tiles * 4096); };
        auto leave = [&](auto V) {
            constexpr int v = V;
#ifndef NTX_X_NOSTORE
            __builtin_amdgcn_raw_buffer_store_b32(__builtin_bit_cast(int, hin[v]), rs_out, lane_o, o_value_bytes(v), STORE_NT);
#endif
        };
        auto bits_leave = [&](int idx, const u32x4 &bw) {
#ifndef NTX_X_NOBITS
            const __amdgpu_buffer_rsrc_t rb = make_rsrc(a.bits + (size_t)idx * a.bits_stride + (size_t)blk * 256, 1024);
            __builtin_amdgcn_raw_buffer_store_b128(__builtin_bit_cast(i32x4, bw), rb, lane16, 0, 0);
#endif
        };
        static_for<8>([&](auto T) { bias_tile<decltype(T)::value>(acc, aux, 0, h); });
        seg_mem<PSG>(acc, ws, sbase, pb, fetch);
        float sig_part = 0.0f;
        auto layer = [&](auto LIc) {
            f32x16 (&cur)[8] = acc; f32x16 (&prev)[8] = acc;
            constexpr int LI = decltype(LIc)::value, in_idx = LI - 1;
            constexpr bool relu_in = in_idx != 8;
            u32x4 bw = {0u, 0u, 0u, 0u};
            if constexpr (HOIST && LI == 9) {
                sbase += (uint32_t)DSG * 8192u;
                static_for<RING>([&](auto I) { ws.r[I] = wr_load(ws, sbase + (uint32_t)decltype(I)::value * 1024u); });
            }
            static_for<4>([&](auto W) {
                constexpr int wd = W;
                if constexpr (relu_in) {
                    uint32_t w = 0;
                    static_for<4>([&](auto Q) { convert8_relu_bits<32 * wd + 8 * decltype(Q)::value>(hin, prev, w); });
                    bw[wd] = w;
                } else static_for<32>([&](auto V) { constexpr int v = 32 * wd + decltype(V)::value; hin[v] = prev[v >> 4][v & 15]; });
                const float *bsrc = (HOIST && LI == 9) ? rows_aux : aux;
                if constexpr (LI < 10 || wd < 2) { bias_tile<2 * wd>(cur, bsrc, LI, h); bias_tile<2 * wd + 1>(cur, bsrc, LI, h); }
            });
            if constexpr (relu_in) bits_leave(in_idx < 8 ? in_idx : 8, bw);
            if constexpr (LI == 8) {
                const f32x4 *wa = reinterpret_cast<const f32x4 *>(aux + AUX_ALPHA_W + h * 128);
                static_for<32>([&](auto I) {
                    constexpr int i = I;
                    const f32x4 w = wa[i];
                    sig_part = __builtin_fmaf(hin[4 * i + 0], w.x, sig_part); sig_part = __builtin_fmaf(hin[4 * i + 1], w.y, sig_part);
                    sig_part = __builtin_fmaf(hin[4 * i + 2], w.z, sig_part); sig_part = __builtin_fmaf(hin[4 * i + 3], w.w, sig_part);
                });
            }
            __builtin_amdgcn_sched_barrier(0);
            leaves_to(in_idx, 8);
            if constexpr (LI == 5) seg_mem<PSG>(cur, ws, sbase, pb, fetch);
            if constexpr (LI == 9 && !HOIST) seg_mem<DSG>(cur, ws, sbase, pb, fetch);
            if constexpr (LI == 4) rs_in = make_rsrc(a.pos + (size_t)blk * a.ptiles * 1024, (long long)a.ptiles * 4096);
            if constexpr (LI == 8 && !HOIST) rs_in = make_rsrc(a.dir + (size_t)blk * a.dtiles * 1024, (long long)a.dtiles * 4096);
            if constexpr (LI == 10) {
                const int nb = blk + nwaves < n_blocks ? blk + nwaves : blk;
                rs_in = make_rsrc(a.pos + (size_t)nb * a.ptiles * 1024, (long long)a.ptiles * 4096);
            }
            auto extra = [&](auto S, auto MT) {
                constexpr int s = decltype(S)::value, mt = decltype(MT)::value;
                if constexpr ((LI == 4 || (LI == 8 && !HOIST) || LI == 10) && mt == 2 && (s == 8 || s == 24)) fetch(std::integral_constant<int, (s == 8 ? 0 : 1)>{});
                if constexpr (mt == 5 || (LI == 10 && mt == 3)) leave(S);
            };
            if constexpr (LI == 10) seg_hidden<128, 4, false>(cur, ws, sbase, hin, extra);
            else seg_hidden<128, 8, false>(cur, ws, sbase, hin, extra);
        };
        static_for<10>([&](auto I) { layer(std::integral_constant<int, decltype(I)::value + 1>{}); });
        {
            u32x4 bw = {0u, 0u, 0u, 0u};
            convert_relu_bits<4>(hin, acc, bw);
            bits_leave(9, bw);
            leaves_to(10, 4);
            static_for<64>([&](auto V) { leave(V); });
            float rgb[3];
            static_for<3>([&](auto C) {
                constexpr int c = C;
                const f32x4 *wc = reinterpret_cast<const f32x4 *>(aux + AUX_RGB_W + (c * 2 + h) * 64);
                float p = 0.0f;
                static_for<16>([&](auto I) {
                    constexpr int i = I;
                    const f32x4 w = wc[i];
                    p = __builtin_fmaf(hin[4 * i + 0], w.x, p); p = __builtin_fmaf(hin[4 * i + 1], w.y, p);
                    p = __builtin_fmaf(hin[4 * i + 2], w.z, p); p = __builtin_fmaf(hin[4 * i + 3], w.w, p);
                });
                rgb[c] = p + __shfl_xor(p, 32, 64) + aux[AUX_RGB_B + c];
            });
            const float sigma = sig_part + __shfl_xor(sig_part, 32, 64) + aux[AUX_ALPHA_B];
            if (valid && h == 0) {
                a.sigma[m] = sigma;
                a.raw_rgb[3 * m + 0] = rgb[0]; a.raw_rgb[3 * m + 1] = rgb[1]; a.raw_rgb[3 * m + 2] = rgb[2];
            }
        }
    }
}

#endif

struct DxArgs {
    const float *stream; uint32_t stream_bytes;
    long long M;
    const float *dgrad;
    float *out; long long out_stride;
    const unsigned int *bits; long long bits_stride;
};

#ifdef NTX_TRAIN_DX
__global__ __launch_bounds__(256) __attribute__((amdgpu_waves_per_eu(1, 1))) void dx_chain_kernel(DxArgs a) {
    const int lane = threadIdx.x & 63, n = lane & 31, h = lane >> 5;
    const int wave = __builtin_amdgcn_readfirstlane(blockIdx.x * 4 + (threadIdx.x >> 6)), nwaves = gridDim.x * 4;
    const int n_blocks = (int)((a.M + 31) >> 5);
    if (wave >= n_blocks) return;
    WRingT<DX_RING> ws;
    ws.rsrc = make_rsrc(a.stream, a.stream_bytes);
    ws.voff = (uint32_t)lane * 16u;
    static_for<DX_RING>([&](auto I) { ws.r[I] = wr_load(ws, (uint32_t)decltype(I)::value * 1024u); });
    const uint32_t lane_o = o_lane_bytes(lane), lane16 = (uint32_t)lane * 16u;
    auto fetch_grad = [&](int blk) {
        const long long m = (long long)blk * 32 + n;
        const f32x4 zero = {0.0f, 0.0f, 0.0f, 0.0f};
        return m < a.M ? *reinterpret_cast<const f32x4 *>(a.dgrad + 4 * m) : zero;
    };
    f32x4 g = fetch_grad(wave);
    for (int blk = wave; blk < n_blocks; blk += nwaves) {
        uint32_t sbase = 0;
        f32x16 acc[8];
        float hin[128];
        __amdgpu_buffer_rsrc_t rs_out = make_rsrc(a.out, 0);
        auto leaves_to = [&](int idx, int tiles) { rs_out = make_rsrc(a.out + (size_t)idx * a.out_stride + (size_t)blk * tiles * 1024, (long long)tiles * 4096); };
        auto leave = [&](auto V) {
            constexpr int v = V;
            __builtin_amdgcn_raw_buffer_store_b32(__builtin_bit_cast(int, hin[v]), rs_out, lane_o, o_value_bytes(v), STORE_NT);
        };
        auto fetch_bits = [&](int idx) {
            const __amdgpu_buffer_rsrc_t rb = make_rsrc(a.bits + (size_t)idx * a.bits_stride + (size_t)blk * 256, 1024);
            return __builtin_bit_cast(u32x4, __builtin_amdgcn_raw_buffer_load_b128(rb, lane16, 0, 0));
        };
        u32x4 bw = fetch_bits(9);
        const float gs = h ? 0.0f : g.w;
        {
            const float b[2] = {h ? g.y : g.x, h ? 0.0f : g.z};
            seg_few<2, 4, true>(acc, ws, sbase, b);
        }
        {
            const int nb = blk + nwaves < n_blocks ? blk + nwaves : blk;
            g = fetch_grad(nb);
        }
        convert_mask<4>(hin, acc, bw);
        bw = fetch_bits(8);
        leaves_to(0, 4);
        seg_hidden<64, 8, true>(acc, ws, sbase, hin, [&](auto S, auto MT) { if constexpr (decltype(MT)::value == 5) leave(S); });
        convert_mask<8>(hin, acc, bw);
        leaves_to(1, 8);
        seg_hidden<128, 8, true>(acc, ws, sbase, hin, [&](auto S, auto MT) { if constexpr (decltype(MT)::value == 5) leave(S); });
        convert_linear<8>(hin, acc);
        static_for<8>([&](auto J) {
            constexpr int j = J;
            bw = fetch_bits(7 - j);
            leaves_to(2 + j, 8);
            seg_hidden<128, 8, true>(acc, ws, sbase, hin, [&](auto S, auto MT) { if constexpr (decltype(MT)::value == 5) leave(S); });
            if constexpr (j == 0) {
                const float b[1] = {gs};
                seg_few<1, 8, false>(acc, ws, sbase, b);
            }
            convert_mask<8>(hin, acc, bw);
        });
        leaves_to(10, 8);
        static_for<128>([&](auto V) { leave(V); });
    }
}

#endif

struct DwWave {
    const float *A; int rtA, a0;
    const float *B; int rtB, b0;
    int shape;
    long long out; int ldc;
    int row0, rows_valid, col0, c_lo, c_hi;
    long long bias_out;
};
struct DwJob { DwWave w[4]; int cost; long long slot_floats, first_float; };
struct DwArgs { const DwJob *jobs; int n_jobs, n_blocks; long long total_cost; float *partial;
                unsigned long long *clocks; };

__host__ __device__ inline long long dw_cut(long long g, long long G, long long W, long long start, long long cost, long long n_blocks) {
    const long long x = g * W / G - start;
    long long b = x <= 0 ? 0 : (x + cost / 2) / cost;
    return b > n_blocks ? n_blocks : b;
}
__host__ __device__ inline long long dw_first_g(long long G, long long W, long long start) { return start * G / W; }
__host__ __device__ inline long long dw_last_g(long long G, long long W, long long start, long long span) { return (start + span - 1) * G / W; }

#ifdef NTX_TRAIN_DW
#ifndef NTX_DW_SYNC
#define NTX_DW_SYNC 16
#endif
constexpr int DW_SYNC = NTX_DW_SYNC;
template <int NA, int NB>
TRN_DEV void dw_piece(const DwWave &tg, float *slot, int blk0, int blk1, int lane) {
    auto uniform_ptr = [](const float *p) {
        const uint32_t lo = (uint32_t)__builtin_amdgcn_readfirstlane((int)(uint32_t)(uintptr_t)p), hi = (uint32_t)__builtin_amdgcn_readfirstlane((int)(uint32_t)((uintptr_t)p >> 32));
        return (const float *)(uintptr_t)(((uint64_t)hi << 32) | (uint64_t)lo);
    };
    const float *A = uniform_ptr(tg.A), *B = uniform_ptr(tg.B);
    const int rtA = __builtin_amdgcn_readfirstlane(tg.rtA), a0 = __builtin_amdgcn_readfirstlane(tg.a0), rtB = __builtin_amdgcn_readfirstlane(tg.rtB), b0 = __builtin_amdgcn_readfirstlane(tg.b0);
    f32x16 acc[NA][NB];
    static_for<NA>([&](auto Ai) { static_for<NB>([&](auto Bi) {
        acc[Ai][Bi] = f32x16{0.f, 0.f, 0.f, 0.f, 0.f, 0.f, 0.f, 0.f, 0.f, 0.f, 0.f, 0.f, 0.f, 0.f, 0.f, 0.f}; }); });
    f32x4 bsum[NB];
    static_for<NB>([&](auto Bi) { bsum[Bi] = f32x4{0.0f, 0.0f, 0.0f, 0.0f}; });
    const bool want_bias = tg.bias_out >= 0;
    const int nblk = blk1 - blk0;
    if (nblk > 0) {
        const __amdgpu_buffer_rsrc_t ra = make_rsrc(A + (size_t)blk0 * rtA * 1024, (long long)nblk * rtA * 4096);
        const __amdgpu_buffer_rsrc_t rb = make_rsrc(B + (size_t)blk0 * rtB * 1024, (long long)nblk * rtB * 4096);
        const uint32_t voff = (uint32_t)lane * 16u;
        const uint32_t stepA = (uint32_t)rtA * 4096u, stepB = (uint32_t)rtB * 4096u, offA = (uint32_t)a0 * 4096u, offB = (uint32_t)b0 * 4096u;
        f32x4 xa[2][NA][2], xb[2][NB][2];
        auto fetch = [&](auto BUF, int i) {
            constexpr int buf = BUF;
#ifdef NTX_X_DWSMALL
            i &= 3;
#endif
#ifdef NTX_X_DWNOLOAD
            if (i > 0) return;
#endif
            const uint32_t oa = (uint32_t)i * stepA + offA + (uint32_t)buf * 2048u, ob = (uint32_t)i * stepB + offB + (uint32_t)buf * 2048u;
            static_for<NA>([&](auto Ai) { static_for<2>([&](auto Q) {
                xa[buf][Ai][Q] = __builtin_bit_cast(f32x4, __builtin_amdgcn_raw_buffer_load_b128(ra, voff, oa + (uint32_t)(decltype(Ai)::value * 4 + decltype(Q)::value) * 1024u, 0)); }); });
            static_for<NB>([&](auto Bi) { static_for<2>([&](auto Q) {
                xb[buf][Bi][Q] = __builtin_bit_cast(f32x4, __builtin_amdgcn_raw_buffer_load_b128(rb, voff, ob + (uint32_t)(decltype(Bi)::value * 4 + decltype(Q)::value) * 1024u, 0)); }); });
        };
        auto compute = [&](auto BUF) {
            constexpr int buf = BUF;
            static_for<2>([&](auto Q) { static_for<4>([&](auto C) {
                constexpr int q = Q, c = C;
                static_for<NA>([&](auto Ai) { static_for<NB>([&](auto Bi) {
                    acc[Ai][Bi] = mfma32(xa[buf][Ai][q][c], xb[buf][Bi][q][c], acc[Ai][Bi]);
                }); });
            }); });
            if (want_bias) static_for<NB>([&](auto Bi) { bsum[Bi] += xb[buf][Bi][0] + xb[buf][Bi][1]; });
        };
        fetch(std::integral_constant<int, 0>{}, 0);
        for (int i = 0; i < nblk; ++i) {
            if ((i & (DW_SYNC - 1)) == 0) __builtin_amdgcn_s_barrier();
            fetch(std::integral_constant<int, 1>{}, i);
            __builtin_amdgcn_sched_barrier(0);
            compute(std::integral_constant<int, 0>{});
            __builtin_amdgcn_sched_barrier(0);
            fetch(std::integral_constant<int, 0>{}, i + 1 < nblk ? i + 1 : i);
            __builtin_amdgcn_sched_barrier(0);
            compute(std::integral_constant<int, 1>{});
            __builtin_amdgcn_sched_barrier(0);
        }
    }
    const int j = lane & 31, hh = lane >> 5;
    const int ldc = __builtin_amdgcn_readfirstlane(tg.ldc), row0 = __builtin_amdgcn_readfirstlane(tg.row0), rows_valid = __builtin_amdgcn_readfirstlane(tg.rows_valid);
    const int col0 = __builtin_amdgcn_readfirstlane(tg.col0), c_lo = __builtin_amdgcn_readfirstlane(tg.c_lo), c_hi = __builtin_amdgcn_readfirstlane(tg.c_hi);
    const long long at_out = (long long)(((uint64_t)(uint32_t)__builtin_amdgcn_readfirstlane((int)(uint32_t)((uint64_t)tg.out >> 32)) << 32) | (uint32_t)__builtin_amdgcn_readfirstlane((int)(uint32_t)(uint64_t)tg.out));
    const __amdgpu_buffer_rsrc_t ro = make_rsrc(slot + at_out, (long long)rows_valid * ldc * 4);
    constexpr uint32_t NOWHERE = 0x7ffffff0u;
    static_for<NB>([&](auto Bi) {
        const int col = col0 + 32 * decltype(Bi)::value + j;
        const bool col_ok = col >= c_lo && col < c_hi;
        const uint32_t coff = (uint32_t)(col - c_lo) * 4u;
        static_for<NA>([&](auto Ai) {
            static_for<16>([&](auto R) {
                constexpr int r = R;
                const int row = row0 + 32 * decltype(Ai)::value + 8 * (r >> 2) + (r & 3) + 4 * hh;
                const uint32_t off = (col_ok && row < rows_valid) ? (uint32_t)(row * ldc) * 4u + coff : NOWHERE;
                __builtin_amdgcn_raw_buffer_store_b32(__builtin_bit_cast(int, (float)acc[Ai][Bi][r]), ro, off, 0, 0);
            });
        });
    });
    if (want_bias) {
        const long long at_bias = (long long)(((uint64_t)(uint32_t)__builtin_amdgcn_readfirstlane((int)(uint32_t)((uint64_t)tg.bias_out >> 32)) << 32) | (uint32_t)__builtin_amdgcn_readfirstlane((int)(uint32_t)(uint64_t)tg.bias_out));
        float *bo = slot + at_bias + (size_t)hh * (c_hi - c_lo);
        static_for<NB>([&](auto Bi) {
            const int col = col0 + 32 * decltype(Bi)::value + j;
            const f32x4 sm = bsum[Bi];
            if (col >= c_lo && col < c_hi) bo[col - c_lo] = (sm.x + sm.y) + (sm.z + sm.w);
        });
    }
}

__global__ __launch_bounds__(256) __attribute__((amdgpu_waves_per_eu(1, 1))) void dw_kernel(DwArgs a) {
    const int lane = threadIdx.x & 63, wave = __builtin_amdgcn_readfirstlane(threadIdx.x >> 6);
    const long long g = blockIdx.x, G = gridDim.x, W = a.total_cost * a.n_blocks;
    long long start = 0;
#ifdef NTX_TRAIN_CLOCKS
    unsigned long long *ck = a.clocks ? a.clocks + (size_t)blockIdx.x * (2 + 3 * a.n_jobs) : nullptr;
    if (ck && threadIdx.x == 0) ck[0] = wall_clock64();
#endif
    for (int jn = 0; jn < a.n_jobs; ++jn) {
        const DwJob &job = a.jobs[jn];
        const long long cost = job.cost, span = cost * a.n_blocks;
        const long long g0 = dw_first_g(G, W, start), g1 = dw_last_g(G, W, start, span);
        if (__builtin_amdgcn_readfirstlane((int)(g >= g0 && g <= g1))) {
            const int blk0 = __builtin_amdgcn_readfirstlane((int)dw_cut(g, G, W, start, cost, a.n_blocks)), blk1 = __builtin_amdgcn_readfirstlane((int)dw_cut(g + 1, G, W, start, cost, a.n_blocks));
            const DwWave &wv = job.w[wave];
            const int shape = __builtin_amdgcn_readfirstlane(wv.shape);
            const int my_slot = __builtin_amdgcn_readfirstlane((int)(g - g0));
            float *slot = a.partial + job.first_float + (long long)my_slot * job.slot_floats;
#ifdef NTX_TRAIN_CLOCKS
            const unsigned long long c0 = wall_clock64();
#endif
            if (shape == 0) dw_piece<4, 4>(wv, slot, blk0, blk1, lane);
            else if (shape == 1) dw_piece<3, 4>(wv, slot, blk0, blk1, lane);
            else if (shape == 2) dw_piece<4, 1>(wv, slot, blk0, blk1, lane);
            else for (int i = 0; i < blk1 - blk0; i += DW_SYNC) __builtin_amdgcn_s_barrier();
#ifdef NTX_TRAIN_CLOCKS
            __syncthreads();
            if (ck && threadIdx.x == 0) { ck[2 + 3 * jn] = (unsigned long long)(blk1 - blk0); ck[3 + 3 * jn] = c0; ck[4 + 3 * jn] = wall_clock64(); }
#endif
        }
        start += span;
    }
#ifdef NTX_TRAIN_CLOCKS
    if (ck && threadIdx.x == 0) ck[1] = wall_clock64();
#endif
}
#endif

constexpr int FWD_VARIANTS[4][2] = {{9, 11}, {9, 8}, {11, 8}, {MAX_PB_GROUPS, MAX_PB_GROUPS}};
void launch_fwd_chain(int variant, bool hoist, hipStream_t st, unsigned grid, const FwdArgs &a);
void launch_dx_chain(hipStream_t st, unsigned grid, const DxArgs &a);
void launch_dw(hipStream_t st, unsigned grid, const DwArgs &a);

}
```

Baseline: 112.6 million ray-samples/s.

## Fold linear feature layer into colour layer C1 in training forward and backward

The feature layer has no activation, so its weights are merged with the feature rows of C1 into a single 256x256 matrix and a combined bias. A small fold kernel builds these before packing, and an unfold kernel maps the gradients of the fused matrix back onto the original feature and C1 weights after the reduction. This removes one 256x256 GEMM layer from the fused forward and dx chains, and one activation/gradient buffer and its dW job. The cost is two extra small launches per step, fp64 accumulation inside them, and the loss of the layer-29 gradient debug output. It also adds an asm clobber of a255, which appears intended to make the chain kernels claim the whole register file.

```diff
diff --git a/nerf_tex_amd/csrc/ntx_train.hip b/nerf_tex_amd/csrc/ntx_train.hip
--- a/nerf_tex_amd/csrc/ntx_train.hip
+++ b/nerf_tex_amd/csrc/ntx_train.hip
@@ -229,6 +229,43 @@
     }
     for (int q = 0; z < r.n_split; ++z, ++q) s4[q] += at(z);
     r.out[e] = (s4[0] + s4[1]) + (s4[2] + s4[3]);
+}
+
+constexpr int MAX_FOLD_JOBS = 3;
+struct FoldJob {
+    const float *A; long long ai, ak;
+    const float *B; long long bk, bj;
+    const float *u, *v, *add;
+    float *C; int rows;
+};
+struct FoldArgs { FoldJob job[MAX_FOLD_JOBS]; };
+__global__ __launch_bounds__(256) void fold_kernel(FoldArgs a) {
+    const FoldJob &J = a.job[blockIdx.z];
+    const int i0 = blockIdx.y * 16, j0 = blockIdx.x * 16;
+    if (i0 >= J.rows) return;
+    __shared__ __attribute__((aligned(16))) float As[16][260], Bs[256][17];
+    const int t = threadIdx.x, ti = t >> 4, tj = t & 15;
+#pragma unroll
+    for (int r = 0; r < 16; ++r) {
+        const int i = J.ak == 1 ? r : (t & 15), k = J.ak == 1 ? t : (t >> 4) + 16 * r;
+        As[i][k] = i0 + i < J.rows ? J.A[(long long)(i0 + i) * J.ai + (long long)k * J.ak] : 0.0f;
+        const int kb = J.bj == 1 ? (t >> 4) + 16 * r : t, j = J.bj == 1 ? (t & 15) : r;
+        Bs[kb][j] = J.B[(long long)kb * J.bk + (long long)(j0 + j) * J.bj];
+    }
+    __syncthreads();
+    const int i = i0 + ti, j = j0 + tj;
+    if (i >= J.rows) return;
+    double s4[4] = {0.0, 0.0, 0.0, 0.0};
+#pragma unroll 8
+    for (int k = 0; k < 256; k += 4) {
+        const f32x4 av = *reinterpret_cast<const f32x4 *>(&As[ti][k]);
+        s4[0] = fma((double)av.x, (double)Bs[k][tj], s4[0]); s4[1] = fma((double)av.y, (double)Bs[k + 1][tj], s4[1]);
+        s4[2] = fma((double)av.z, (double)Bs[k + 2][tj], s4[2]); s4[3] = fma((double)av.w, (double)Bs[k + 3][tj], s4[3]);
+    }
+    double acc = (s4[0] + s4[1]) + (s4[2] + s4[3]);
+    if (J.u) acc = fma((double)J.u[i], (double)J.v[j], acc);
+    if (J.add) acc += (double)J.add[j];
+    J.C[(size_t)i * 256 + j] = (float)acc;
 }
 
 enum { PACK_HIDDEN = 0, PACK_LINEAR = 1, PACK_AUX_ROW = 2, PACK_AUX_RGB = 3, PACK_COPY = 4 };
@@ -538,6 +575,8 @@
     long long cap = 0, cap_blocks = 0, cap_rays = 0;
     float *w = nullptr, *grad = nullptr, *adam_m = nullptr, *adam_v = nullptr;
     float *wfwd = nullptr, *wdx = nullptr, *aux = nullptr; size_t fwd_floats = 0, dx_floats = 0;
+    float *wfold = nullptr, *bfold = nullptr, *fold_m = nullptr;
+    ntx_train::FoldArgs fold{}, unfold{};
     ntx_train::PackSeg *pack_seg = nullptr; int n_pack = 0; long long pack_total = 0;
     float *posO = nullptr, *dirO = nullptr;
     float *act = nullptr; long long act_stride = 0;
@@ -564,7 +603,7 @@
 void free_all(ntx_trainer *t) {
     if (!t) return;
     (void)hipSetDevice(t->device);
-    void *ptrs[] = {t->w, t->grad, t->adam_m, t->adam_v, t->wfwd, t->wdx, t->aux, t->pack_seg, t->posO, t->dirO, t->sigma, t->raw_rgb, t->z, t->dists, t->noise,
+    void *ptrs[] = {t->w, t->grad, t->adam_m, t->adam_v, t->wfwd, t->wdx, t->aux, t->wfold, t->bfold, t->fold_m, t->pack_seg, t->posO, t->dirO, t->sigma, t->raw_rgb, t->z, t->dists, t->noise,
                     t->dgrad, t->dhead, t->jobs, t->dw_partial, t->stash, t->dirrow, t->color, t->alpha_out, t->ray_loss, t->loss, t->act, t->bits, t->gout};
     for (void *p : ptrs) if (p) (void)hipFree(p);
     delete t;
@@ -653,7 +692,8 @@
     alloc(&t->w, p); alloc(&t->grad, p, true); alloc(&t->adam_m, p, true); alloc(&t->adam_v, p, true);
     alloc(&t->posO, (size_t)NB * t->ptiles * 1024, true); alloc(&t->dirO, (size_t)NB * t->dtiles * 1024, true);
     t->act_stride = t->gout_stride = NB * 8 * 1024; t->bits_stride = NB * 256;
-    alloc(&t->act, (size_t)t->act_stride * 11); alloc((float **)&t->bits, (size_t)t->bits_stride * 10); alloc(&t->gout, (size_t)t->gout_stride * 11);
+    alloc(&t->act, (size_t)t->act_stride * 10); alloc((float **)&t->bits, (size_t)t->bits_stride * 10); alloc(&t->gout, (size_t)t->gout_stride * 10);
+    alloc(&t->wfold, 256 * 256, true); alloc(&t->bfold, 256, true); alloc(&t->fold_m, 256 * 256, true);
     auto act = [&](int i) { return t->act + (size_t)i * t->act_stride; };
     auto gout = [&](int i) { return t->gout + (size_t)i * t->gout_stride; };
     alloc(&t->sigma, (size_t)M); alloc(&t->raw_rgb, (size_t)M * 3); alloc(&t->z, (size_t)(M + max_rays)); alloc(&t->dists, (size_t)M); alloc(&t->noise, (size_t)M);
@@ -679,15 +719,14 @@
         if (i == 5) { fwd_linear(t->trunk[5], Kp, t->PS); fwd_hidden(t->trunk[5], Kp, 8); }
         else fwd_hidden(t->trunk[i], 0, 8);
     }
-    fwd_hidden(t->feature, 0, 8);
-    fwd_linear(t->c1, Kd, t->DS); fwd_hidden(t->c1, Kd, 8);
+    fwd_linear(t->c1, Kd, t->DS);
+    seg(t->wfold, 256, 1, PACK_HIDDEN, 256, 256, 8, &t->fwd_floats, 128);
     fwd_hidden(t->c2, 0, 4);
     const size_t n_fwd_segs = segs.size();
     auto dx_hidden = [&](const TLayer &l, int row0, int K, int nsteps) { seg(W + l.w + (size_t)row0 * l.out, 1, l.out, PACK_HIDDEN, K, 256, 8, &t->dx_floats, nsteps); };
     seg(W + t->rgb.w, 1, 3, PACK_LINEAR, 3, 128, 4, &t->dx_floats, 2);
     dx_hidden(t->c2, 0, 128, 64);
-    dx_hidden(t->c1, Kd, 256, 128);
-    dx_hidden(t->feature, 0, 256, 128);
+    seg(t->wfold, 1, 256, PACK_HIDDEN, 256, 256, 8, &t->dx_floats, 128);
     seg(W + t->alpha.w, 1, 1, PACK_LINEAR, 1, 256, 8, &t->dx_floats, 1);
     for (int i = 7; i >= 1; --i) dx_hidden(t->trunk[i], i == 5 ? Kp : 0, 256, 128);
     const size_t n_stream_segs = segs.size();
@@ -699,8 +738,8 @@
         first += count; segs.push_back(s);
     };
     for (int i = 0; i < 8; ++i) aux_seg(W + t->trunk[i].b, PACK_AUX_ROW, 256, 256, AUX_BIAS + (size_t)i * 256);
-    aux_seg(W + t->feature.b, PACK_AUX_ROW, 256, 256, AUX_BIAS + 8 * 256); aux_seg(W + t->c1.b, PACK_AUX_ROW, 256, 256, AUX_BIAS + 9 * 256);
-    aux_seg(W + t->c2.b, PACK_AUX_ROW, 128, 256, AUX_BIAS + 10 * 256);
+    aux_seg(t->bfold, PACK_AUX_ROW, 256, 256, AUX_BIAS + 8 * 256);
+    aux_seg(W + t->c2.b, PACK_AUX_ROW, 128, 256, AUX_BIAS + 9 * 256);
     aux_seg(W + t->alpha.w, PACK_AUX_ROW, 256, 256, AUX_ALPHA_W); aux_seg(W + t->alpha.b, PACK_COPY, 1, 1, AUX_ALPHA_B);
     aux_seg(W + t->rgb.w, PACK_AUX_RGB, 128, 384, AUX_RGB_W); aux_seg(W + t->rgb.b, PACK_COPY, 3, 3, AUX_RGB_B);
     t->pack_total = first; t->n_pack = (int)segs.size();
@@ -716,17 +755,18 @@
             rc = ntx_set_error(NTX_E_HIP, "segment table upload failed");
     }
     std::vector<DwJob> &jobs = t->jobs_host;
-    struct RJ { int job; long long at, count, pair; size_t out; };
+    struct RJ { int job; long long at, count, pair; float *out; };
     std::vector<RJ> rjobs;
     auto new_job = [&]() { DwJob j{}; for (DwWave &w : j.w) w.shape = -1; jobs.push_back(j); return (int)jobs.size() - 1; };
-    auto matrix = [&](int j, int K, int N, size_t g_kernel, long long g_bias, long long *at_bias) {
+    auto matrix_to = [&](int j, int K, int N, float *kernel_out, long long g_bias, long long *at_bias) {
         const long long at = jobs[j].slot_floats;
         jobs[j].slot_floats += (long long)K * N;
-        rjobs.push_back(RJ{j, at, (long long)K * N, 0, g_kernel});
+        rjobs.push_back(RJ{j, at, (long long)K * N, 0, kernel_out});
         *at_bias = -1;
-        if (g_bias >= 0) { *at_bias = jobs[j].slot_floats; jobs[j].slot_floats += 2 * N; rjobs.push_back(RJ{j, *at_bias, N, N, (size_t)g_bias}); }
+        if (g_bias >= 0) { *at_bias = jobs[j].slot_floats; jobs[j].slot_floats += 2 * N; rjobs.push_back(RJ{j, *at_bias, N, N, t->grad + g_bias}); }
         return at;
     };
+    auto matrix = [&](int j, int K, int N, size_t g_kernel, long long g_bias, long long *at_bias) { return matrix_to(j, K, N, t->grad + g_kernel, g_bias, at_bias); };
     auto wave = [&](int j, int w, int shape, const float *A, int rtA, int a0, const float *B, int rtB, int b0, long long at, int K, int N, int c_lo, long long at_bias) {
         DwWave &d = jobs[j].w[w];
         d.A = A; d.rtA = rtA; d.a0 = a0; d.B = B; d.rtB = rtB; d.b0 = b0; d.shape = shape; d.out = at; d.ldc = N; d.row0 = a0 * 32; d.rows_valid = K;
@@ -734,29 +774,28 @@
         const int cost = shape == 0 ? 256 : shape == 1 ? 198 : 68;
         if (cost > jobs[j].cost) jobs[j].cost = cost;
     };
-    auto layer_job = [&](const float *X, const float *dY, size_t g_kernel, size_t g_bias) {
-        const int j = new_job(); long long ab; const long long at = matrix(j, 256, 256, g_kernel, (long long)g_bias, &ab);
+    auto layer_job = [&](const float *X, const float *dY, float *kernel_out, size_t g_bias) {
+        const int j = new_job(); long long ab; const long long at = matrix_to(j, 256, 256, kernel_out, (long long)g_bias, &ab);
         for (int w = 0; w < 4; ++w) wave(j, w, 0, X, 8, 4 * (w >> 1), dY, 8, 4 * (w & 1), at, 256, 256, 0, ab);
     };
     {
-        const TLayer &r = t->rgb, &al = t->alpha, &c2 = t->c2, &c1 = t->c1, &f = t->feature;
-        for (int i = 7; i >= 1; --i) layer_job(act(i - 1), gout(10 - i), t->trunk[i].w + (size_t)(i == 5 ? Kp : 0) * 256, t->trunk[i].b);
-        layer_job(act(7), gout(2), f.w, f.b);
-        layer_job(act(8), gout(1), c1.w + (size_t)Kd * 256, c1.b);
+        const TLayer &r = t->rgb, &al = t->alpha, &c2 = t->c2, &c1 = t->c1;
+        for (int i = 7; i >= 1; --i) layer_job(act(i - 1), gout(9 - i), t->grad + t->trunk[i].w + (size_t)(i == 5 ? Kp : 0) * 256, t->trunk[i].b);
+        layer_job(act(7), gout(1), t->fold_m, c1.b);
         {
             const int j = new_job(); long long ab0, ab5;
             const long long at0 = matrix(j, Kp, 256, t->trunk[0].w, (long long)t->trunk[0].b, &ab0), at5 = matrix(j, Kp, 256, t->trunk[5].w, -1, &ab5);
-            for (int w = 0; w < 2; ++w) { wave(j, w, 1, t->posO, t->ptiles, 0, gout(10), 8, 4 * w, at0, Kp, 256, 0, ab0); wave(j, 2 + w, 1, t->posO, t->ptiles, 0, gout(5), 8, 4 * w, at5, Kp, 256, 0, ab5); }
+            for (int w = 0; w < 2; ++w) { wave(j, w, 1, t->posO, t->ptiles, 0, gout(9), 8, 4 * w, at0, Kp, 256, 0, ab0); wave(j, 2 + w, 1, t->posO, t->ptiles, 0, gout(4), 8, 4 * w, at5, Kp, 256, 0, ab5); }
         }
         {
             const int j = new_job(); long long abd, ab2;
             const long long atd = matrix(j, Kd, 256, c1.w, -1, &abd), at2 = matrix(j, 256, 128, c2.w, (long long)c2.b, &ab2);
-            for (int w = 0; w < 2; ++w) { wave(j, w, 1, t->dirO, t->dtiles, 0, gout(1), 8, 4 * w, atd, Kd, 256, 0, abd); wave(j, 2 + w, 0, act(9), 8, 4 * w, gout(0), 4, 0, at2, 256, 128, 0, ab2); }
+            for (int w = 0; w < 2; ++w) { wave(j, w, 1, t->dirO, t->dtiles, 0, gout(1), 8, 4 * w, atd, Kd, 256, 0, abd); wave(j, 2 + w, 0, act(8), 8, 4 * w, gout(0), 4, 0, at2, 256, 128, 0, ab2); }
         }
         {
             const int j = new_job(); long long abr, aba;
             const long long atr = matrix(j, 128, 3, r.w, (long long)r.b, &abr), ata = matrix(j, 256, 1, al.w, (long long)al.b, &aba);
-            wave(j, 0, 2, act(10), 4, 0, t->dhead, 1, 0, atr, 128, 3, 0, abr);
+            wave(j, 0, 2, act(9), 4, 0, t->dhead, 1, 0, atr, 128, 3, 0, abr);
             for (int w = 0; w < 2; ++w) wave(j, 1 + w, 2, act(7), 8, 4 * w, t->dhead, 1, 0, ata, 256, 1, 3, aba);
         }
     }
@@ -780,12 +819,25 @@
             ReduceJob &r = t->reduce.job[t->reduce.n++];
             const DwJob &j = jobs[rjobs[i].job];
             r.partial = t->dw_partial + j.first_float + rjobs[i].at; r.n_split = 0; r.stride = j.slot_floats; r.count = rjobs[i].count; r.pair = rjobs[i].pair;
-            r.out = t->grad + rjobs[i].out; r.first = rfirst;
+            r.out = rjobs[i].out; r.first = rfirst;
             rfirst += (rjobs[i].count + 255) / 256 * 256;
             t->reduce_job.push_back(rjobs[i].job);
         }
     }
     if (rc != NTX_OK) { free_all(t); return rc; }
+    {
+        const TLayer &f = t->feature, &c1 = t->c1;
+        const float *Wf = t->w + f.w, *bf = t->w + f.b, *Wcf = t->w + c1.w + (size_t)Kd * 256, *bc = t->w + c1.b, *s = t->grad + c1.b;
+        auto job = [](const float *A, long long ai, long long ak, const float *B, long long bk, long long bj, float *C, int rows) {
+            FoldJob j{}; j.A = A; j.ai = ai; j.ak = ak; j.B = B; j.bk = bk; j.bj = bj; j.C = C; j.rows = rows; return j;
+        };
+        t->fold.job[0] = job(Wf, 256, 1, Wcf, 256, 1, t->wfold, 256);
+        t->fold.job[1] = job(bf, 0, 1, Wcf, 256, 1, t->bfold, 1); t->fold.job[1].add = bc;
+        t->unfold.job[0] = job(t->fold_m, 256, 1, Wcf, 1, 256, t->grad + f.w, 256);
+        t->unfold.job[1] = job(s, 0, 1, Wcf, 1, 256, t->grad + f.b, 1);
+        t->unfold.job[2] = job(Wf, 1, 256, t->fold_m, 256, 1, t->grad + c1.w + (size_t)Kd * 256, 256);
+        t->unfold.job[2].u = bf; t->unfold.job[2].v = s;
+    }
     *out = t;
     return NTX_OK;
 }
@@ -816,15 +868,17 @@
     auto act = [&](int i) { return t->act + (size_t)i * t->act_stride; };
     auto gout = [&](int i) { return t->gout + (size_t)i * t->gout_stride; };
     if (layer >= 0 && layer < 8) src = act(layer);
-    else if (layer == 8) src = act(9);
-    else if (layer == 9) { src = act(10); tiles = 4; }
+    else if (layer == 8) src = act(8);
+    else if (layer == 9) { src = act(9); tiles = 4; }
     else if (layer == 10) src = t->sigma;
-    else if (layer >= 20 && layer < 28) src = gout(10 - (layer - 20));
+    else if (layer >= 20 && layer < 28) src = gout(9 - (layer - 20));
     else if (layer == 28) src = gout(1);
-    else if (layer == 29) src = gout(2);
+    else if (layer == 29)
+        return ntx_set_error(NTX_E_UNSUPPORTED, "layer 29 (the gradient at the feature layer's output) is never formed: the training step runs the linear feature layer "
+                                                "folded into the colour layer C1 (W_fold = W_feature . W_C1[feature rows]); its weight gradients are in the gradient blob");
     else if (layer == 11) src = t->raw_rgb;
     else if (layer == 30) src = t->dgrad;
-    else return ntx_set_error(NTX_E_INVALID, "layer %d (0-7 trunk, 8 / 9 the colour layers, 10 the density, 11 the raw colour; 20-29 the kept gradients, 30 the composite's adjoint)", layer);
+    else return ntx_set_error(NTX_E_INVALID, "layer %d (0-7 trunk, 8 / 9 the colour layers, 10 the density, 11 the raw colour; 20-28 the kept gradients, 30 the composite's adjoint)", layer);
     TRAIN_TRY(hipSetDevice(t->device));
     TRAIN_TRY(hipDeviceSynchronize());
     if (layer == 10 || layer == 11 || layer == 30) {
@@ -922,6 +976,7 @@
     const long long M = (long long)n_rays * n_samples;
     const int S = n_samples, n_blocks = (int)((M + 31) / 32);
     {
+        hipLaunchKernelGGL(fold_kernel, dim3(16, 16, 2), dim3(256), 0, st, t->fold);
         PackArgs pa{t->pack_seg, t->n_pack, t->pack_total};
         hipLaunchKernelGGL(pack_kernel, dim3((unsigned)((t->pack_total + 255) / 256)), dim3(256), 0, st, pa);
     }
@@ -954,7 +1009,7 @@
         const bool hoist = (t->ipe || blur_idx < 0 || blur_idx < t->desc.n_geo) && S % 32 == 0 && getenv("NERFTEX_TRAIN_NO_DIR_HOIST") == nullptr;
         if (hoist) {
             DirRowArgs dr{}; dr.rays_d = rays_d; dr.params = params; dr.rays_per_param_row = rays_per_param_row; dr.n_rays = (int)n_rays; dr.n_geo = t->desc.n_geo;
-            dr.n_app = t->desc.n_app; dr.dir_freq = t->desc.dir_freq; dr.param_freq = t->desc.param_freq; dr.Kd = t->Kd; dr.w = t->w + t->c1.w; dr.bias = t->w + t->c1.b;
+            dr.n_app = t->desc.n_app; dr.dir_freq = t->desc.dir_freq; dr.param_freq = t->desc.param_freq; dr.Kd = t->Kd; dr.w = t->w + t->c1.w; dr.bias = t->bfold;
             dr.rows = t->dirrow; dr.splice = t->ipe ? blur_idx : -1;
             hipLaunchKernelGGL(dirrow_kernel, dim3((unsigned)n_rays), dim3(256), 0, st, dr);
         }
@@ -1021,6 +1076,7 @@
         for (int i = 0; i < rb.n; ++i) rb.job[i].n_split = slots[t->reduce_job[i]];
         const long long total = rb.job[rb.n - 1].first + (rb.job[rb.n - 1].count + 255) / 256 * 256;
         hipLaunchKernelGGL(reduce_batch_kernel, dim3((unsigned)(total / 256)), dim3(256), 0, st, rb);
+        hipLaunchKernelGGL(fold_kernel, dim3(16, 16, 3), dim3(256), 0, st, t->unfold);
     }
     TRAIN_TRY(hipGetLastError());
     return NTX_OK;
diff --git a/nerf_tex_amd/csrc/ntx_train_device.h b/nerf_tex_amd/csrc/ntx_train_device.h
--- a/nerf_tex_amd/csrc/ntx_train_device.h
+++ b/nerf_tex_amd/csrc/ntx_train_device.h
@@ -147,10 +147,6 @@
     });
 }
 template <int NMT>
-TRN_DEV void convert_linear(float (&hin)[128], const f32x16 (&prev)[8]) {
-    static_for<NMT * 16>([&](auto V) { constexpr int v = V; hin[v] = prev[v >> 4][v & 15]; });
-}
-template <int NMT>
 TRN_DEV void convert_mask(float (&hin)[128], const f32x16 (&prev)[8], const u32x4 &bits) {
     static_for<NMT * 16>([&](auto V) {
         constexpr int v = V;
@@ -160,7 +156,7 @@
     });
 }
 
-constexpr int AUX_BIAS = 0, AUX_ALPHA_W = 11 * 256, AUX_ALPHA_B = AUX_ALPHA_W + 256, AUX_RGB_W = AUX_ALPHA_B + 4, AUX_RGB_B = AUX_RGB_W + 384,
+constexpr int AUX_BIAS = 0, AUX_ALPHA_W = 10 * 256, AUX_ALPHA_B = AUX_ALPHA_W + 256, AUX_RGB_W = AUX_ALPHA_B + 4, AUX_RGB_B = AUX_RGB_W + 384,
               AUX_FLOATS = AUX_RGB_B + 4;
 template <int MT>
 TRN_DEV void bias_tile(f32x16 (&acc)[8], const float *aux, int layer, int h) {
@@ -168,6 +164,8 @@
     const f32x4 v0 = b[0], v1 = b[1], v2 = b[2], v3 = b[3];
     acc[MT] = f32x16{v0.x, v0.y, v0.z, v0.w, v1.x, v1.y, v1.z, v1.w, v2.x, v2.y, v2.z, v2.w, v3.x, v3.y, v3.z, v3.w};
 }
+
+TRN_DEV void whole_register_file() { asm volatile("" ::: "a255"); }
 
 constexpr int MAX_PB_GROUPS = 12;
 struct FwdArgs {
@@ -185,6 +183,7 @@
 #ifdef NTX_TRAIN_FWD
 template <int PSG, int DSG, bool HOIST>
 __global__ __launch_bounds__(256) __attribute__((amdgpu_waves_per_eu(1, 1))) void fwd_chain_kernel(FwdArgs a) {
+    whole_register_file();
     __shared__ __attribute__((aligned(16))) float aux_lds[AUX_FLOATS];
     __shared__ __attribute__((aligned(16))) float rows_lds[HOIST ? 4 * 256 : 4];
     ntx::load_aux(aux_lds, a.aux, AUX_FLOATS);
@@ -213,7 +212,7 @@
         uint32_t opaque_zero = 0;
         asm volatile("" : "+v"(opaque_zero));
         const float *aux = aux_lds + opaque_zero;
-        const float *rows_aux = rows_lds + opaque_zero + (HOIST ? (threadIdx.x >> 6) * 256 : 0) - AUX_BIAS - 9 * 256;
+        const float *rows_aux = rows_lds + opaque_zero + (HOIST ? (threadIdx.x >> 6) * 256 : 0) - AUX_BIAS - 8 * 256;
         uint32_t sbase = 0;
         f32x16 acc[8];
         float hin[128];
@@ -245,23 +244,20 @@
         auto layer = [&](auto LIc) {
             f32x16 (&cur)[8] = acc; f32x16 (&prev)[8] = acc;
             constexpr int LI = decltype(LIc)::value, in_idx = LI - 1;
-            constexpr bool relu_in = in_idx != 8;
             u32x4 bw = {0u, 0u, 0u, 0u};
-            if constexpr (HOIST && LI == 9) {
+            if constexpr (HOIST && LI == 8) {
                 sbase += (uint32_t)DSG * 8192u;
                 static_for<RING>([&](auto I) { ws.r[I] = wr_load(ws, sbase + (uint32_t)decltype(I)::value * 1024u); });
             }
             static_for<4>([&](auto W) {
                 constexpr int wd = W;
-                if constexpr (relu_in) {
-                    uint32_t w = 0;
-                    static_for<4>([&](auto Q) { convert8_relu_bits<32 * wd + 8 * decltype(Q)::value>(hin, prev, w); });
-                    bw[wd] = w;
-                } else static_for<32>([&](auto V) { constexpr int v = 32 * wd + decltype(V)::value; hin[v] = prev[v >> 4][v & 15]; });
-                const float *bsrc = (HOIST && LI == 9) ? rows_aux : aux;
-                if constexpr (LI < 10 || wd < 2) { bias_tile<2 * wd>(cur, bsrc, LI, h); bias_tile<2 * wd + 1>(cur, bsrc, LI, h); }
+                uint32_t w = 0;
+                static_for<4>([&](auto Q) { convert8_relu_bits<32 * wd + 8 * decltype(Q)::value>(hin, prev, w); });
+                bw[wd] = w;
+                const float *bsrc = (HOIST && LI == 8) ? rows_aux : aux;
+                if constexpr (LI < 9 || wd < 2) { bias_tile<2 * wd>(cur, bsrc, LI, h); bias_tile<2 * wd + 1>(cur, bsrc, LI, h); }
             });
-            if constexpr (relu_in) bits_leave(in_idx < 8 ? in_idx : 8, bw);
+            bits_leave(in_idx, bw);
             if constexpr (LI == 8) {
                 const f32x4 *wa = reinterpret_cast<const f32x4 *>(aux + AUX_ALPHA_W + h * 128);
                 static_for<32>([&](auto I) {
@@ -274,27 +270,27 @@
             __builtin_amdgcn_sched_barrier(0);
             leaves_to(in_idx, 8);
             if constexpr (LI == 5) seg_mem<PSG>(cur, ws, sbase, pb, fetch);
-            if constexpr (LI == 9 && !HOIST) seg_mem<DSG>(cur, ws, sbase, pb, fetch);
+            if constexpr (LI == 8 && !HOIST) seg_mem<DSG>(cur, ws, sbase, pb, fetch);
             if constexpr (LI == 4) rs_in = make_rsrc(a.pos + (size_t)blk * a.ptiles * 1024, (long long)a.ptiles * 4096);
-            if constexpr (LI == 8 && !HOIST) rs_in = make_rsrc(a.dir + (size_t)blk * a.dtiles * 1024, (long long)a.dtiles * 4096);
-            if constexpr (LI == 10) {
+            if constexpr (LI == 7 && !HOIST) rs_in = make_rsrc(a.dir + (size_t)blk * a.dtiles * 1024, (long long)a.dtiles * 4096);
+            if constexpr (LI == 9) {
                 const int nb = blk + nwaves < n_blocks ? blk + nwaves : blk;
                 rs_in = make_rsrc(a.pos + (size_t)nb * a.ptiles * 1024, (long long)a.ptiles * 4096);
             }
             auto extra = [&](auto S, auto MT) {
                 constexpr int s = decltype(S)::value, mt = decltype(MT)::value;
-                if constexpr ((LI == 4 || (LI == 8 && !HOIST) || LI == 10) && mt == 2 && (s == 8 || s == 24)) fetch(std::integral_constant<int, (s == 8 ? 0 : 1)>{});
-                if constexpr (mt == 5 || (LI == 10 && mt == 3)) leave(S);
+                if constexpr ((LI == 4 || (LI == 7 && !HOIST) || LI == 9) && mt == 2 && (s == 8 || s == 24)) fetch(std::integral_constant<int, (s == 8 ? 0 : 1)>{});
+                if constexpr (mt == 5 || (LI == 9 && mt == 3)) leave(S);
             };
-            if constexpr (LI == 10) seg_hidden<128, 4, false>(cur, ws, sbase, hin, extra);
+            if constexpr (LI == 9) seg_hidden<128, 4, false>(cur, ws, sbase, hin, extra);
             else seg_hidden<128, 8, false>(cur, ws, sbase, hin, extra);
         };
-        static_for<10>([&](auto I) { layer(std::integral_constant<int, decltype(I)::value + 1>{}); });
+        static_for<9>([&](auto I) { layer(std::integral_constant<int, decltype(I)::value + 1>{}); });
         {
             u32x4 bw = {0u, 0u, 0u, 0u};
             convert_relu_bits<4>(hin, acc, bw);
             bits_leave(9, bw);
-            leaves_to(10, 4);
+            leaves_to(9, 4);
             static_for<64>([&](auto V) { leave(V); });
             float rgb[3];
             static_for<3>([&](auto C) {
@@ -330,6 +326,7 @@
 
 #ifdef NTX_TRAIN_DX
 __global__ __launch_bounds__(256) __attribute__((amdgpu_waves_per_eu(1, 1))) void dx_chain_kernel(DxArgs a) {
+    whole_register_file();
     const int lane = threadIdx.x & 63, n = lane & 31, h = lane >> 5;
     const int wave = __builtin_amdgcn_readfirstlane(blockIdx.x * 4 + (threadIdx.x >> 6)), nwaves = gridDim.x * 4;
     const int n_blocks = (int)((a.M + 31) >> 5);
@@ -374,13 +371,10 @@
         leaves_to(0, 4);
         seg_hidden<64, 8, true>(acc, ws, sbase, hin, [&](auto S, auto MT) { if constexpr (decltype(MT)::value == 5) leave(S); });
         convert_mask<8>(hin, acc, bw);
-        leaves_to(1, 8);
-        seg_hidden<128, 8, true>(acc, ws, sbase, hin, [&](auto S, auto MT) { if constexpr (decltype(MT)::value == 5) leave(S); });
-        convert_linear<8>(hin, acc);
         static_for<8>([&](auto J) {
             constexpr int j = J;
             bw = fetch_bits(7 - j);
-            leaves_to(2 + j, 8);
+            leaves_to(1 + j, 8);
             seg_hidden<128, 8, true>(acc, ws, sbase, hin, [&](auto S, auto MT) { if constexpr (decltype(MT)::value == 5) leave(S); });
             if constexpr (j == 0) {
                 const float b[1] = {gs};
@@ -388,7 +382,7 @@
             }
             convert_mask<8>(hin, acc, bw);
         });
-        leaves_to(10, 8);
+        leaves_to(9, 8);
         static_for<128>([&](auto V) { leave(V); });
     }
 }
```

Result: no change. 112.7 million ray-samples/s (median of 6 runs) (+0.2%).
